# TomBeacock/volumetric-renderer

Hardware: AMD Instinct MI355X
Metric: Gsamples/sec + fps, 512³ NRRD @ 1080p; achieved HBM GB/s vs peak (higher is better)
Workload: dtype f32

## Files before the change

include/vr/vr.h:

```cpp
#ifndef VR_VR_H
#define VR_VR_H

#include <stddef.h>
#include <stdint.h>

#ifdef __cplusplus
extern "C" {
#endif

#define VR_ABI_VERSION 9

#define VR_OK 0
#define VR_EINVAL (-22)
#define VR_ENOMEM (-12)
#define VR_ENODEV (-19)
#define VR_ENODATA (-61)
#define VR_EIO (-5)

enum vr_dtype {
    VR_DTYPE_I8 = 1,
    VR_DTYPE_U8 = 2,
    VR_DTYPE_I16 = 3,
    VR_DTYPE_U16 = 4,
    VR_DTYPE_I32 = 5,
// ... 31 lines not shown
    int32_t skip_empty;
    int32_t wave_shape;
    int32_t frames_in_flight;
    int32_t exact_gradient;
    int32_t depth_zero_to_one;
} vr_params;

typedef struct vr_stats {
    uint64_t rays;
    uint64_t samples;
    uint64_t shaded_samples;
    uint64_t steps;
    uint64_t skipped_samples;
} vr_stats;

int vr_abi_version(void);
void vr_params_default(vr_params *p);

typedef struct vr_ctx vr_ctx;
vr_ctx *vr_create(int device, uint32_t width, uint32_t height);
vr_ctx *vr_create_mask(uint32_t device_mask, uint32_t width, uint32_t height);
void vr_destroy(vr_ctx *ctx);
const char *vr_last_error(const vr_ctx *ctx);

int vr_resize(vr_ctx *ctx, uint32_t width, uint32_t height);
int vr_get_size(const vr_ctx *ctx, uint32_t *width, uint32_t *height);
int vr_get_device(const vr_ctx *ctx, int *device);
int vr_get_device_mask(const vr_ctx *ctx, uint32_t *device_mask);


int vr_set_volume(vr_ctx *ctx, const void *data, int dtype, uint32_t nx, uint32_t ny,
                  uint32_t nz, float vmin, float vmax);
int vr_set_volume_device(vr_ctx *ctx, const void *data_dev, int dtype, uint32_t nx,
                         uint32_t ny, uint32_t nz, float vmin, float vmax, void *stream);
int vr_generate_volume(vr_ctx *ctx, int kind, int dtype, uint32_t nx, uint32_t ny,
                       uint32_t nz, uint32_t seed, float *vmin_out, float *vmax_out);
uint64_t vr_volume_bytes(const vr_ctx *ctx);
int vr_debug_read_volume(vr_ctx *ctx, float *out_host);
int vr_debug_read_volume_native(vr_ctx *ctx, void *out_host);
int vr_debug_volume_info(const vr_ctx *ctx, uint32_t dims[3], float minmax[2], int *storage);

int vr_set_transfer_function(vr_ctx *ctx, const uint32_t *rgba8_srgb, uint32_t n);

int vr_set_slicing(vr_ctx *ctx, const float min_slice[3], const float max_slice[3]);


int vr_render(vr_ctx *ctx, const vr_camera *cam, const vr_params *p, void *out,
              int out_format);

int vr_render_device(vr_ctx *ctx, const vr_camera *cam, const vr_params *p, void *out_dev,
                     int out_format, uint32_t row_block, uint32_t rank, uint32_t nranks,
                     void *stream);
uint32_t vr_shard_rows(uint32_t height, uint32_t row_block, uint32_t nranks);
int vr_set_row_share(vr_ctx *ctx, uint32_t first_weight, uint32_t other_weight);
int vr_get_row_share(const vr_ctx *ctx, uint32_t *first_weight, uint32_t *other_weight);
uint32_t vr_shard_rows_ctx(const vr_ctx *ctx, uint32_t height, uint32_t row_block, uint32_t nranks);
int vr_assemble_rows(vr_ctx *ctx, const void *gathered_dev, void *out_dev, int out_format,
                     uint32_t row_block, uint32_t nranks, void *stream);

typedef struct vr_external_memory vr_external_memory;
int vr_import_memory_fd(vr_ctx *ctx, int fd, uint64_t size, uint64_t offset,
                        vr_external_memory **mem, void **dev_ptr);
int vr_release_external_memory(vr_ctx *ctx, vr_external_memory *mem);

typedef struct vr_memory_info {
    uint64_t volume_bytes;
    uint64_t field_bytes;
    uint64_t oblique_copy_bytes;
    uint64_t plain_copy_bytes;
    uint64_t stencil_copy_bytes;
    uint64_t skip_bytes;
    uint64_t derived_bytes;
    uint64_t budget_bytes;
    uint64_t builds;
    uint64_t evictions;
    uint64_t downgrades;
    uint64_t last_downgrade;
} vr_memory_info;
enum vr_derived {
    VR_DERIVED_FIELD = 1,
    VR_DERIVED_OBLIQUE_COPY = 2,
    VR_DERIVED_PLAIN_COPY = 3,
    VR_DERIVED_STENCIL_COPY = 4,
    VR_DERIVED_SKIP = 5
};
#define VR_MEMORY_BUDGET_UNLIMITED (~(uint64_t)0)
#define VR_MEMORY_BUDGET_DEFAULT (~(uint64_t)0 - 1)
int vr_set_memory_budget(vr_ctx *ctx, uint64_t bytes);
int vr_memory_report(const vr_ctx *ctx, vr_memory_info *out);
int vr_prepare(vr_ctx *ctx, const vr_camera *cam, const vr_params *p);

int vr_count_work(vr_ctx *ctx, const vr_camera *cam, const vr_params *p, uint32_t row_block,
                  uint32_t rank, uint32_t nranks, vr_stats *out);

int vr_timing_enable(vr_ctx *ctx, int enable);
int vr_timing_read(vr_ctx *ctx, double *total_ms, uint64_t *launches);
int vr_timing_reset(vr_ctx *ctx);

const char *vr_kernel_name(const vr_ctx *ctx, const vr_params *p);

#ifdef __cplusplus
}
#endif

#endif
```

include/vr/vr_debug.h:

```cpp
#ifndef VR_VR_DEBUG_H
#define VR_VR_DEBUG_H

#include "vr.h"
#include "vr_dist.h"

#ifdef __cplusplus
extern "C" {
#endif

enum vr_knob {
    VR_KNOB_PIPELINE = 1,
    VR_KNOB_PAIR = 2,
    VR_KNOB_PAIR_LANES = 3,
    VR_KNOB_GRAD_FIELD = 4,
    VR_KNOB_U8_LAYOUT = 6,
    VR_KNOB_TILE_ORDER = 7,
    VR_KNOB_NARROW = 8,
    VR_KNOB_ALT_GEOMETRY = 9,
    VR_KNOB_MIP_INFLIGHT = 10
};

typedef struct vr_member_timing {
    int32_t device;
    uint64_t frames;
    double kernel_ms, render_ms, gather_ms, assemble_ms;
} vr_member_timing;
int vr_debug_timing_member(vr_ctx *ctx, int member, vr_member_timing *out);

enum vr_exchange { VR_EXCHANGE_RCCL = 0, VR_EXCHANGE_COPY = 1 };
vr_ctx *vr_debug_create_members(const int *devices, int n, uint32_t width, uint32_t height,
                                int exchange);
int vr_debug_fail_member(vr_ctx *ctx, int member, uint64_t frame);

int vr_debug_host_profile_enable(vr_ctx *ctx, int enable);
int vr_debug_host_profile_member(vr_ctx *ctx, int member, vr_dist_host_profile *out);

int vr_debug_set_knob(vr_ctx *ctx, int knob, int value);
int vr_debug_get_knob(const vr_ctx *ctx, int knob, int *value);

typedef struct vr_variant_facts {
    int32_t layout, mode;
    int32_t shade, count, skip, field, field_half, pipeline;
    int32_t tf_n, pair, mip_inflight;
} vr_variant_facts;
int vr_debug_variant_name(const vr_variant_facts *facts, char *buf, size_t n);
const char *vr_debug_last_kernel_name(const vr_ctx *ctx);

#ifdef __cplusplus
}
#endif

#endif
```

volumetric-renderer_amd/csrc/vr_api.hip:

```cpp
#include "../../include/vr/vr.h"
#include "../../include/vr/vr_debug.h"
#include "../../include/vr/vr_modes.h"
#include "../../include/vr/vr_iso.h"
#include "vr_internal.h"
#include "vr_group.h"

#include <algorithm>
#include <cmath>
#include <cstdio>
#include <cstdlib>
#include <cstring>
#include <new>
#include <string>
#include <vector>

#pragma clang fp contract(off)

using namespace vr;

#ifndef VR_HOST_BANDS
#define VR_HOST_BANDS 4
#endif
constexpr int kRenderBands = VR_HOST_BANDS;

struct vr_ctx {
    int device = 0;
    uint32_t width = 0, height = 0;
    void *bricks = nullptr;
    size_t brick_bytes = 0;
    int storage = ST_F32;
    int layout = ST_F32;
    bool dense_rows = false;
    double pixel_span = 0.0;
    double axis_align = 1.0;
    int ray_axis = 2;
    double row_align = 1.0;
    struct AltCopy {
        void *bricks = nullptr;
        size_t bytes = 0;
        bool valid = false, failed = false;
        uint64_t used = 0;
    } alt[3];
    uint32_t nx = 1, ny = 1, nz = 1;
    float vmin = 0.0f, vmax = 1.0f;
    float4 *tf = nullptr;
    uint32_t tf_n = 0;
    uint32_t *tf_nz = nullptr;
    float smin[3] = {0.0f, 0.0f, 0.0f};
    float smax[3] = {1.0f, 1.0f, 1.0f};
    int render_mode = VR_MODE_COMPOSITE;
    float isovalue = 0.0f;
    float2 *brick_range = nullptr;
    uint8_t *skip_dist = nullptr;
    size_t nbricks_alloc = 0;
    bool range_valid = false, dist_valid = false;
    float *grad = nullptr;
    size_t grad_bytes = 0;
    bool grad_valid = false;
    uint64_t grad_used = 0;
    bool grad_half = false;
    int grad_scale_log2 = 0;
    float data_lo = 0.0f, data_hi = 1.0f;
    struct TileSched {
        uint32_t tiles_x = 0, tiles_y = 0, supers_x = 0, per_xcd = 0;
        uint32_t row_block = 0, rank = 0, nranks = 0, share_w0 = 1, share_w = 1;
        int pair = 0;
        uint32_t kernel = 0;
        void *stream = nullptr;
        uint32_t *cost = nullptr, *perm = nullptr, *lists = nullptr;
        bool have_perm = false;
        uint32_t launches = 0;
    };
    std::vector<TileSched> sched;
    hipEvent_t built_ev = nullptr;
    bool built_recorded = false;
    struct Fence {
        hipStream_t stream;
        hipEvent_t ev;
        uint64_t used;
        bool external;
        uint64_t build_seen;
    };
    std::vector<Fence> fences;
    uint64_t build_gen = 0;
    uint64_t frame_no = 0;
    FrameVariant last_variant;
    uint64_t n_builds = 0, n_evictions = 0, n_downgrades = 0;
    uint32_t last_downgrade = 0;
    unsigned long long *counters = nullptr;
    void *frame_dev = nullptr;
    size_t frame_bytes = 0;
    hipStream_t band_stream[2] = {nullptr, nullptr};
    hipStream_t copy_stream = nullptr;
    hipEvent_t band_ev[kRenderBands] = {};
    bool timing = false;
    std::vector<hipEvent_t> ev_pool;
    std::vector<std::pair<hipEvent_t, hipEvent_t>> ev_pending;
    double timed_ms = 0.0;
    uint64_t timed_launches = 0;
    struct Knobs {
        int pipeline = -1, pair = -1, pair_lanes = 0, grad_field = -1, u8_layout = -1,
            tile_order = 0, narrow = 1, alt = -1, mip_inflight = 0;
    } knobs;
    std::vector<vr_ctx *> members;
    vr::Group *group = nullptr;
    uint32_t device_mask = 0;
    hipStream_t group_stream = nullptr;
    RowShare share{1, 1};
    uint64_t budget = VR_MEMORY_BUDGET_DEFAULT;
    std::string err;
};

namespace {

thread_local std::string g_err;

int fail(vr_ctx *c, int code, const std::string &msg)
{
    if (c)
        c->err = msg;
    else
        g_err = msg;
    return code;
}

// ... 312 lines not shown
}

int check_params(vr_ctx *c, const vr_params *p)
{
    if (!p) return fail(c, VR_EINVAL, "params is NULL");
    if (!(p->step > 0.0f) || !std::isfinite(p->step))
        return fail(c, VR_EINVAL, "params.step must be a positive finite float");
    if (!(p->ray_dist >= 0.0f) || !std::isfinite(p->ray_dist))
        return fail(c, VR_EINVAL, "params.ray_dist must be finite and >= 0");
    if (p->spec_power < 0 || p->spec_power > 256)
        return fail(c, VR_EINVAL, "params.spec_power must be in [0, 256]");
    if (p->frames_in_flight < 0 || p->frames_in_flight > 16)
        return fail(c, VR_EINVAL, "params.frames_in_flight must be in [0, 16]");
    if (p->exact_gradient != 0 && p->exact_gradient != 1)
        return fail(c, VR_EINVAL, "params.exact_gradient must be 0 or 1");
    if (p->depth_zero_to_one != 0 && p->depth_zero_to_one != 1)
        return fail(c, VR_EINVAL, "params.depth_zero_to_one must be 0 or 1");
    const float n = p->ray_dist / p->step;
    if (n > 1.0e8f) return fail(c, VR_EINVAL, "params.ray_dist / step too large");
    return VR_OK;
}

bool view_dense_rows(const double *inv, uint32_t W, uint32_t nx, uint32_t ny, uint32_t nz,
                     double *span, double *align, int *axis, double *row_align)
{
    *span = 0.0;
    *align = 1.0;
    *axis = 2;
    *row_align = 1.0;
    auto unproject = [&](double x, double z, double out[3]) {
        double h[4];
        for (int r = 0; r < 4; ++r) h[r] = inv[0 * 4 + r] * x + inv[2 * 4 + r] * z + inv[3 * 4 + r];
        for (int a = 0; a < 3; ++a) out[a] = h[a] / h[3];
    };
    double o[3], f[3], o2[3], f2[3], d[3], s[3];
    unproject(0.0, 0.0, o);
    unproject(0.0, 1.0, f);
    const double dx = 2.0 / (double)W;
    unproject(dx, 0.0, o2);
    unproject(dx, 1.0, f2);
    double od = 0.0, dd = 0.0;
    for (int a = 0; a < 3; ++a) {
        d[a] = f[a] - o[a];
        od += o[a] * d[a];
        dd += d[a] * d[a];
    }
    if (!(dd > 0.0)) return false;
    *align = std::fmax(std::fabs(d[0]), std::fmax(std::fabs(d[1]), std::fabs(d[2]))) / std::sqrt(dd);
    *axis = std::fabs(d[0]) >= std::fabs(d[1]) ? (std::fabs(d[0]) >= std::fabs(d[2]) ? 0 : 2)
                                               : (std::fabs(d[1]) >= std::fabs(d[2]) ? 1 : 2);
    const double t = -od / dd;
    double n2 = 0.0, v2 = 0.0;
    const double nv[3] = {(double)nx, (double)ny, (double)nz};
    for (int a = 0; a < 3; ++a) {
        s[a] = (o2[a] + t * (f2[a] - o2[a])) - (o[a] + t * d[a]);
        n2 += s[a] * s[a];
        v2 += (s[a] * nv[a]) * (s[a] * nv[a]);
    }
    if (!(n2 > 0.0)) return false;
    *span = std::sqrt(v2);
    *row_align = std::fabs(s[0]) / std::sqrt(n2);
    return *row_align >= 0.9 && *span <= 0.8;
}

constexpr double kAltAlign = 0.9, kAltSpan = 0.8, kRowsAlign = 0.97;
bool use_grad_field(const vr_ctx *c, bool half)
{
    if (c->storage != ST_F32) return false;
    if (c->knobs.grad_field >= 0) return c->knobs.grad_field == 1;
    if (c->dense_rows) return true;
    if (!half || c->axis_align < kAltAlign || c->ray_axis == 0) return false;
    return c->pixel_span <= kAltSpan || (c->ray_axis == 2 && c->row_align >= kRowsAlign);
}

bool use_pipeline(bool shading, uint32_t tiles, const vr_ctx *c)
{
    if (c->knobs.pipeline >= 0) return c->knobs.pipeline == 1;
    const size_t voxels = (size_t)c->nx * c->ny * c->nz;
    return tiles * (kThreadsPerTile / 64) < kPipelineMaxWaves ||
           c->brick_bytes >= kPipelineMinBytes || voxels >= kPipelineMinVoxels || c->dense_rows ||
           (shading && c->storage == ST_F32);
}

int want_alt(const vr_ctx *c, const vr_params *p, bool pair, bool field);
bool use_pair(const vr_ctx *c, const MarchParams &P, const vr_params *p)
{
    if (p->skip_empty || P.tf_n > kTfLds) return false;
    if (c->knobs.pair >= 0) return c->knobs.pair == 1;
    if (p->frames_in_flight >= 2) return false;
    if (!p->shading) return false;
    if (P.tiles_x * P.tiles_y * (kThreadsPerTile / 64) < kPairMaxWaves) return true;
    if (c->knobs.alt >= 0 || c->layout != ST_F32 || c->dense_rows || c->pixel_span <= kAltSpan ||
        (c->ray_axis == 2 && c->axis_align >= kAltAlign))
        return false;
    return want_alt(c, p, P.pair != 0, P.grad != nullptr) == (ST_F32 | kAltFlag);
}

int build_params(vr_ctx *c, const vr_camera *cam, const vr_params *p, void *out,
                 int out_format, uint32_t row_block, uint32_t rank, uint32_t nranks,
                 RowShare share, MarchParams &P)
{
    if (!cam) return fail(c, VR_EINVAL, "camera is NULL");
    int rc = check_params(c, p);
    if (rc) return rc;
    if (out_format != VR_OUT_RGBA8 && out_format != VR_OUT_RGBA32F)
        return fail(c, VR_EINVAL, "unknown out_format");
    if (nranks == 0 || rank >= nranks || row_block == 0)
        return fail(c, VR_EINVAL, "bad shard (row_block, rank, nranks)");
    std::memset(&P, 0, sizeof(P));
    if (!unprojection(cam, c->width, c->height, p->depth_zero_to_one != 0, P.inv))
        return fail(c, VR_EINVAL, "proj * view is singular");
    P.vol = c->bricks;
    P.vol_bytes = c->brick_bytes;
    P.tf = c->tf;
    P.out = out;
    P.counters = c->counters;
    P.fw = (double)c->width;
    P.fh = (double)c->height;
    P.nx = c->nx;
    P.ny = c->ny;
    P.nz = c->nz;
    P.nbx = bricks_for(c->nx, 0, c->layout);
    P.nby = bricks_for(c->ny, 1, c->layout);
    P.fnx = (float)c->nx;
    P.fny = (float)c->ny;
    P.fnz = (float)c->nz;
    P.vmin = c->vmin;
    P.range = c->vmax - c->vmin;
    P.div_fast = P.range >= 0x1p-40f && P.range < 0x1p100f && std::fabs(c->vmin) < 0x1p100f &&
                 std::fabs(c->vmax) < 0x1p100f;
    P.inv_range = P.div_fast ? 1.0f / P.range : 0.0f;
    P.tf_n = (int32_t)c->tf_n;
    P.tf_nf = (float)c->tf_n;
    for (int a = 0; a < 3; ++a) {
        P.smin[a] = c->smin[a];
        P.smax[a] = c->smax[a];
        P.cam[a] = cam->position[a];
    }
    P.step = p->step;
    P.nsteps = (int32_t)(p->ray_dist / p->step);
    P.ert_eps = p->ert_eps;
    for (int k = 0; k < 4; ++k) P.clear[k] = p->clear_color[k];
    P.ka = p->ambient;
    P.kd = p->diffuse;
    P.ks = p->specular;
    P.spec_power = p->spec_power;
    P.W = c->width;
    P.H = c->height;
    P.row_block = row_block;
    P.rank = rank;
    P.nranks = nranks;
    P.local_rows = share_shard_rows(c->height, row_block, nranks, share);
    P.out_bytes = (unsigned long long)P.local_rows * c->width * (out_format == VR_OUT_RGBA32F ? 16 : 4);
    P.share_w0 = share.w0;
    P.share_w = share.w;
    P.tiles_x = (c->width + 15) / 16;
    P.tiles_y = (P.local_rows + kMarchRows - 1) / kMarchRows;
    P.tile_order = p->tile_order >= 1 && p->tile_order <= 4 ? (uint32_t)p->tile_order : 4u;
    if (p->tile_order == 0 && c->knobs.tile_order >= 1)
        P.tile_order = (uint32_t)c->knobs.tile_order;
    P.wave_w_shift = p->wave_shape == 1 ? 3u : (p->wave_shape == 3 ? 2u : 4u);
    while ((64u >> P.wave_w_shift) > kMarchRows) ++P.wave_w_shift;
    P.supers_x = (P.tiles_x + kSuper - 1) / kSuper;
    P.supers_total = P.supers_x * ((P.tiles_y + kSuper - 1) / kSuper);
    P.out_format = out_format;
    P.slab_default = c->smin[0] == 0.0f && c->smin[1] == 0.0f && c->smin[2] == 0.0f &&
                     c->smax[0] == 1.0f && c->smax[1] == 1.0f && c->smax[2] == 1.0f;
    c->dense_rows = view_dense_rows(P.inv, c->width, c->nx, c->ny, c->nz, &c->pixel_span,
                                    &c->axis_align, &c->ray_axis, &c->row_align);
    P.pipelined = use_pipeline(p->shading != 0, P.tiles_x * P.tiles_y, c);
    return VR_OK;
}

vr_ctx::Fence *fence_of(vr_ctx *c, hipStream_t s)
{
    for (auto &x : c->fences)
        if (x.stream == s) return &x;
    return nullptr;
// ... 6 lines not shown
    c->built_recorded = true;
    ++c->build_gen;
    if (vr_ctx::Fence *f = fence_of(c, s)) f->build_seen = c->build_gen;
    return VR_OK;
}

constexpr size_t kSkipBytesPerBrick = sizeof(float2) + 2;
size_t derived_bytes(const vr_ctx *c)
{
    size_t b = c->grad ? c->grad_bytes : 0;
    for (const auto &a : c->alt)
        if (a.bricks) b += a.bytes + kBrickSlackBytes;
    return b + c->nbricks_alloc * kSkipBytesPerBrick;
}
constexpr uint64_t kDerivedBudgetBricks = 5;
uint64_t effective_budget(const vr_ctx *c)
{
    if (c->budget != VR_MEMORY_BUDGET_DEFAULT) return c->budget;
    return kDerivedBudgetBricks * (uint64_t)c->brick_bytes + (uint64_t)c->brick_bytes / 32 +
           64ull * kBrickSlackBytes;
}
bool budget_allows(const vr_ctx *c, size_t extra, size_t replaced)
{
    if (c->budget == VR_MEMORY_BUDGET_UNLIMITED) return true;
    const size_t now = derived_bytes(c) - replaced;
    return now + extra <= effective_budget(c);
}
constexpr size_t kMaxFences = 32;
#ifndef VR_FENCE_SYSTEM_SCOPE
#define VR_FENCE_SYSTEM_SCOPE 0
#endif
constexpr unsigned kFenceEventFlags =
    hipEventDisableTiming | (VR_FENCE_SYSTEM_SCOPE ? 0u : (unsigned)hipEventDisableSystemFence);
int fence_record(vr_ctx *c, hipStream_t s)
{
    vr_ctx::Fence *f = fence_of(c, s);
    if (f && f->external) {
        f->used = c->frame_no;
        return VR_OK;
    }
    if (!f) {
        if (c->fences.size() < kMaxFences) {
            hipEvent_t e = nullptr;
            HIP_TRY(c, hipEventCreateWithFlags(&e, kFenceEventFlags), "hipEventCreate(fence)");
            c->fences.push_back(vr_ctx::Fence{s, e, 0, false, 0});
            f = &c->fences.back();
        } else {
            vr_ctx::Fence *old = nullptr;
            for (auto &x : c->fences)
                if (!x.external && (!old || x.used < old->used)) old = &x;
            if (!old) return VR_OK;
            HIP_TRY(c, hipEventSynchronize(old->ev), "hipEventSynchronize(fence)");
            old->stream = s;
            old->build_seen = 0;
            f = old;
        }
    }
    f->used = c->frame_no;
    HIP_TRY(c, hipEventRecord(f->ev, s), "hipEventRecord(fence)");
    return VR_OK;
}
int fence_others(vr_ctx *c, hipStream_t s)
{
    for (const auto &x : c->fences)
        if (x.stream != s && hipStreamWaitEvent(s, x.ev, 0) != hipSuccess) {
            (void)hipGetLastError();
            HIP_TRY(c, hipDeviceSynchronize(), "hipDeviceSynchronize (fence fallback)");
            for (size_t i = c->fences.size(); i-- > 0;)
                if (!c->fences[i].external) {
                    hipEventDestroy(c->fences[i].ev);
                    c->fences.erase(c->fences.begin() + (long)i);
                }
            return VR_OK;
        }
    return VR_OK;
}
int release_async(vr_ctx *c, void *p, hipStream_t s)
{
    if (!p) return VR_OK;
    if (int rc = fence_others(c, s)) return rc;
    HIP_TRY(c, hipFreeAsync(p, s), "hipFreeAsync(derived structure)");
    return VR_OK;
}
int make_room(vr_ctx *c, size_t extra, size_t replaced, int keep_alt, bool keep_field, hipStream_t s,
              bool *fits)
{
    *fits = budget_allows(c, extra, replaced);
    while (!*fits) {
        int pick = -2;
        uint64_t oldest = ~0ull;
        if (c->grad && !keep_field && c->grad_used < oldest) {
            pick = -1;
            oldest = c->grad_used;
        }
        for (int i = 0; i < (int)(sizeof c->alt / sizeof c->alt[0]); ++i)
            if (i != keep_alt && c->alt[i].bricks && c->alt[i].used < oldest) {
                pick = i;
                oldest = c->alt[i].used;
            }
        if (pick == -2) return VR_OK;
        if (pick == -1) {
            if (int rc = release_async(c, c->grad, s)) return rc;
            c->grad = nullptr;
            c->grad_bytes = 0;
            c->grad_valid = false;
        } else {
            if (int rc = release_async(c, c->alt[pick].bricks, s)) return rc;
            c->alt[pick] = vr_ctx::AltCopy();
        }
        ++c->n_evictions;
        *fits = budget_allows(c, extra, replaced);
    }
    return VR_OK;
}
void free_derived(vr_ctx *c)
{
    if (c->grad) (void)hipFreeAsync(c->grad, nullptr);
    c->grad = nullptr;
    c->grad_bytes = 0;
    c->grad_valid = false;
    for (auto &a : c->alt) {
        if (a.bricks) (void)hipFreeAsync(a.bricks, nullptr);
        a = vr_ctx::AltCopy();
    }
    if (c->brick_range) hipFree(c->brick_range);
    if (c->skip_dist) hipFree(c->skip_dist);
    c->brick_range = nullptr;
    c->skip_dist = nullptr;
    c->nbricks_alloc = 0;
    c->range_valid = c->dist_valid = false;
    (void)hipStreamSynchronize(nullptr);
}

int alloc_skip(vr_ctx *c, size_t nb, bool *have)
{
    *have = false;
    if (nb > 0xFFFFFFFFull) return fail(c, VR_EINVAL, "skip_empty: too many bricks");
    if (c->nbricks_alloc != nb && !budget_allows(c, nb * kSkipBytesPerBrick, c->nbricks_alloc * kSkipBytesPerBrick))
        return VR_OK;
    if (c->nbricks_alloc != nb) {
        if (c->brick_range) hipFree(c->brick_range);
        if (c->skip_dist) hipFree(c->skip_dist);
        c->brick_range = nullptr;
        c->skip_dist = nullptr;
        c->nbricks_alloc = 0;
        c->range_valid = c->dist_valid = false;
        HIP_TRY(c, hipMalloc(&c->brick_range, (nb + 1) * sizeof(float2)), "hipMalloc(brick ranges)");
        HIP_TRY(c, hipMalloc(&c->skip_dist, 2 * nb), "hipMalloc(skip distance field)");
        c->nbricks_alloc = nb;
    }
    *have = true;
    return VR_OK;
}
int build_ranges(vr_ctx *c, size_t nb, hipStream_t s)
{
    if (c->range_valid) return VR_OK;
    HIP_TRY(c, launch_brick_range(c->layout, c->bricks, bricks_for(c->nx, 0, c->layout), bricks_for(c->ny, 1, c->layout),
                                  bricks_for(c->nz, 2, c->layout), c->brick_range, s),
            "brick range kernel");
    HIP_TRY(c, launch_range_max(c->brick_range, (uint32_t)nb, s), "brick range maximum kernel");
    c->range_valid = true;
    c->dist_valid = false;
    return VR_OK;
}
size_t brick_count(const vr_ctx *c)
{
    return (size_t)bricks_for(c->nx, 0, c->layout) * bricks_for(c->ny, 1, c->layout) * bricks_for(c->nz, 2, c->layout);
}

int ensure_skip(vr_ctx *c, MarchParams &P, hipStream_t s)
{
    const size_t nb = brick_count(c);
    bool have = false;
    if (int rc = alloc_skip(c, nb, &have)) return rc;
    if (!have) return VR_OK;
    if (!c->range_valid || !c->dist_valid) ++c->n_builds;
    if (int rc = build_ranges(c, nb, s)) return rc;
    if (!c->dist_valid) {
        HIP_TRY(c, launch_skip_dist(c->brick_range, bricks_for(c->nx, 0, c->layout), bricks_for(c->ny, 1, c->layout),
                                    bricks_for(c->nz, 2, c->layout), c->tf_nz, (int)c->tf_n, c->vmin,
                                    c->vmax - c->vmin, c->skip_dist, c->skip_dist + nb, s),
                "skip distance kernels");
// ... 55 lines not shown
        if (launch_grad_field(static_cast<const float *>(c->bricks), c->grad, c->nx, c->ny, c->nz,
                              half, k, s) != hipSuccess)
            return built;
        built = true;
        ++c->n_builds;
        c->grad_valid = true;
        c->grad_half = half;
        c->grad_scale_log2 = k;
    }
    *refused = false;
    P.grad = c->grad;
    P.grad_half = half ? 1 : 0;
    c->grad_used = c->frame_no;
    return built;
}

int wait_builds(vr_ctx *c, hipStream_t s)
{
    if (c->built_recorded) {
        vr_ctx::Fence *f = fence_of(c, s);
        if (!f || f->build_seen != c->build_gen) {
            HIP_TRY(c, hipStreamWaitEvent(s, c->built_ev, 0), "hipStreamWaitEvent(build)");
            if (f) f->build_seen = c->build_gen;
        }
    }
    return VR_OK;
}
int ensure_derived(vr_ctx *c, const vr_params *p, MarchParams &P, hipStream_t s, uint32_t *refused)
{
    if (int rc = wait_builds(c, s)) return rc;
    const bool r0 = c->range_valid, d0 = c->dist_valid;
    if (p->skip_empty) {
        int rc = ensure_skip(c, P, s);
        if (rc) return rc;
        if (!P.skip_empty) *refused = VR_DERIVED_SKIP;
    }
    bool g_refused = false;
    const bool g_built = p->shading && ensure_grad(c, P, s, p->exact_gradient == 0, &g_refused);
    if (g_refused) *refused = VR_DERIVED_FIELD;
    const bool built = (!r0 && c->range_valid) || (!d0 && c->dist_valid) || g_built;
    if (built) return record_build(c, s);
    return VR_OK;
}

int ensure_mip(vr_ctx *c, const vr_params *p, MarchParams &P, MipArgs &M, hipStream_t s,
               uint32_t *refused)
{
    if (int rc = wait_builds(c, s)) return rc;
    M.brick_range = nullptr;
    M.nbricks = 0;
    P.pipelined = 0;
    if (!p->skip_empty) return VR_OK;
    const bool r0 = c->range_valid;
    if (int rc = ensure_mip_ranges(c, P, M, s)) return rc;
    if (!P.skip_empty) *refused = VR_DERIVED_SKIP;
    if (!r0 && c->range_valid) return record_build(c, s);
    return VR_OK;
}
int mip_inflight(const vr_ctx *c, bool skip)
{
    if (c->knobs.mip_inflight) return c->knobs.mip_inflight;
    if (c->layout == ST_F32 && c->pixel_span > kAltSpan) return skip ? 4 : 1;
    if ((c->layout & kQuadFlag) && skip) return 4;
    return kMipDefaultInFlight;
}

int iso_inflight(const vr_ctx *c, bool skip)
{
    if (c->knobs.mip_inflight) return c->knobs.mip_inflight;
    if (c->layout == ST_F32 && c->pixel_span > kAltSpan) return skip ? 4 : 1;
    if (c->layout == ST_U16 || c->layout == ST_I16) return mip_inflight(c, skip);
    if (c->layout & kQuadFlag) return 4;
    return skip ? 2 : 4;
}
bool range_mode(const vr_ctx *c)
{
    return c->render_mode == VR_MODE_MIP || c->render_mode == VR_MODE_ISO;
}
IsoArgs iso_args(const vr_ctx *c, const vr_params *p, const MipArgs &M)
{
    return {M.brick_range, M.nbricks, c->isovalue, p->shading != 0};
}

int want_alt(const vr_ctx *c, const vr_params *p, bool pair, bool field)
{
    if (c->layout != ST_F32 || p->skip_empty || pair || field) return c->layout;
    int which = 0;
    if (c->knobs.alt >= 0)
        which = c->knobs.alt;
    else if (!c->dense_rows) {
        if (c->pixel_span > kAltSpan && c->row_align >= kRowsAlign)
            which = p->shading ? 4 : 3;
        else if (c->axis_align >= kAltAlign && c->ray_axis != 0 && c->pixel_span <= kAltSpan)
            which = 0;
        else
            which = 1;
    }
    switch (which) {
        case 1: return ST_F32 | kAltFlag;
        case 3: return ST_F32 | kPlainF32Flag;
        case 4: return ST_F32 | kStencilF32Flag;
        default: return c->layout;
    }
}

int alt_index(int layout)
{
    if (layout & kAltFlag) return 0;
    return (layout & kPlainF32Flag) ? 1 : 2;
}

size_t alt_bytes_for(const vr_ctx *c, int lay)
{
    return (size_t)bricks_for(c->nx, 0, lay) * bricks_for(c->ny, 1, lay) * bricks_for(c->nz, 2, lay) *
           brick_elems(lay) * element_size(lay);
}

int ensure_alt(vr_ctx *c, int lay, hipStream_t s, bool *ready)
{
    *ready = false;
    vr_ctx::AltCopy &a = c->alt[alt_index(lay)];
    const size_t bytes = alt_bytes_for(c, lay);
    if (a.valid && a.bricks && a.bytes == bytes) {
        *ready = true;
        a.used = c->frame_no;
        return VR_OK;
    }
    if (a.failed) return VR_OK;
    if (!a.bricks || a.bytes != bytes) {
        const size_t had = a.bricks ? a.bytes + kBrickSlackBytes : 0;
        bool fits = false;
        if (int rc = make_room(c, bytes + kBrickSlackBytes, had, alt_index(lay), false, s, &fits))
            return rc;
        if (!fits) return VR_OK;
        if (int rc = release_async(c, a.bricks, s)) return rc;
        a.bricks = nullptr;
        a.bytes = 0;
        size_t free_b = 0, total_b = 0;
        if (hipMemGetInfo(&free_b, &total_b) != hipSuccess ||
            free_b < bytes + kBrickSlackBytes + (2ull << 30) ||
            hipMallocAsync(&a.bricks, bytes + kBrickSlackBytes, s) != hipSuccess) {
            (void)hipGetLastError();
            a.bricks = nullptr;
            a.failed = true;
            return VR_OK;
        }
        a.bytes = bytes;
    }
    const hipError_t e = launch_rebrick_f32(static_cast<const float *>(c->bricks), a.bricks, c->nx,
                                            c->ny, c->nz, lay, s);
    if (e != hipSuccess) return hip_fail(c, e, "alt geometry copy");
    a.valid = true;
    a.used = c->frame_no;
    ++c->n_builds;
    *ready = true;
    return record_build(c, s);
}

VariantFacts launch_facts(const vr_ctx *c, const vr_params *p, const MarchParams &P, int layout,
                          bool count)
{
    const bool skip = P.skip_empty != 0;
    const int k = c->render_mode == VR_MODE_MIP   ? mip_inflight(c, skip)
                  : c->render_mode == VR_MODE_ISO ? iso_inflight(c, skip)
                                                  : 0;
    return {layout, c->render_mode, p->shading != 0, count, skip, P.grad != nullptr, P.grad_half,
            P.pipelined, P.tf_n, P.pair, k};
}
VariantFacts next_frame_facts(const vr_ctx *c, const vr_params *p)
{
    VariantFacts f{};
    f.layout = c->layout;
    f.mode = c->render_mode;
    f.shade = p && p->shading;
    f.tf_n = (int32_t)c->tf_n;
    if (range_mode(c)) {
        f.skip = p && p->skip_empty && c->range_valid && c->nbricks_alloc;
        f.mip_inflight = f.mode == VR_MODE_ISO ? iso_inflight(c, f.skip) : mip_inflight(c, f.skip);
        return f;
    }
    f.skip = p && p->skip_empty;
    f.field = f.shade && use_grad_field(c, p->exact_gradient == 0) && c->grad && c->grad_valid;
    f.field_half = f.field && p->exact_gradient == 0;
    const uint32_t tiles = ((c->width + 15) / 16) * ((c->height + kMarchRows - 1) / kMarchRows);
    f.pipeline = use_pipeline(f.shade, tiles, c);
    if (p && !f.field)
        if (const int lay = want_alt(c, p, false, false);
            lay != c->layout && c->alt[alt_index(lay)].valid)
            f.layout = lay;
    return f;
}

vr_ctx::TileSched *tile_sched(vr_ctx *c, MarchParams &P, void *stream, uint32_t kernel)
{
    if (P.tile_order != 4) return nullptr;
    auto use = [&P](vr_ctx::TileSched &t) {
        P.tile_cost = t.cost;
        if (t.have_perm) {
            P.tile_perm = t.perm;
            P.nperm = 8 * t.per_xcd;
        }
    };
    for (auto &t : c->sched)
        if (t.tiles_x == P.tiles_x && t.tiles_y == P.tiles_y && t.pair == P.pair &&
            t.kernel == kernel &&
            t.stream == stream && t.row_block == P.row_block && t.rank == P.rank &&
            t.nranks == P.nranks && t.share_w0 == P.share_w0 && t.share_w == P.share_w) {
            use(t);
            return &t;
        }
    if (c->sched.size() >= kMaxTileScheds) {
        hipFree(c->sched.front().cost);
        hipFree(c->sched.front().perm);
        hipFree(c->sched.front().lists);
        c->sched.erase(c->sched.begin());
    }
    vr_ctx::TileSched t;
    t.tiles_x = P.tiles_x;
    t.tiles_y = P.tiles_y;
    t.supers_x = P.supers_x;
    t.pair = P.pair;
    t.kernel = kernel;
    t.stream = stream;
    t.row_block = P.row_block;
    t.rank = P.rank;
    t.nranks = P.nranks;
    t.share_w0 = P.share_w0;
    t.share_w = P.share_w;
    std::vector<std::vector<uint32_t>> xl(8);
    if (VR_LIST_ORDER == 1) {
        const uint32_t sy_n = (P.tiles_y + kSuper - 1) / kSuper;
        for (uint32_t sy = 0; sy < sy_n; ++sy)
            for (uint32_t sx = 0; sx < P.supers_x; ++sx)
                for (uint32_t w = 0; w < kSuper * kSuper; ++w) {
                    const uint32_t tx = sx * kSuper + w % kSuper, ty = sy * kSuper + w / kSuper;
                    if (tx < P.tiles_x && ty < P.tiles_y)
                        xl[(sy * P.supers_x + sx) & 7u].push_back(ty * P.tiles_x + tx);
                }
    } else {
        for (uint32_t ty = 0; ty < P.tiles_y; ++ty)
            for (uint32_t tx = 0; tx < P.tiles_x; ++tx)
                xl[((ty >> kSuperShift) * P.supers_x + (tx >> kSuperShift)) & 7u].push_back(
                    ty * P.tiles_x + tx);
    }
    for (int x = 0; x < 8; ++x) t.per_xcd = xl[x].size() > t.per_xcd ? (uint32_t)xl[x].size() : t.per_xcd;
    std::vector<uint32_t> lists(8 * (size_t)t.per_xcd, 0xFFFFFFFFu);
    for (int x = 0; x < 8; ++x)
        std::copy(xl[x].begin(), xl[x].end(), lists.begin() + (size_t)x * t.per_xcd);
    const size_t nt = (size_t)P.tiles_x * P.tiles_y;
    hipStream_t hs = static_cast<hipStream_t>(stream);
    if (hipMalloc(&t.cost, nt * sizeof(uint32_t)) != hipSuccess ||
        hipMalloc(&t.perm, lists.size() * sizeof(uint32_t)) != hipSuccess ||
        hipMalloc(&t.lists, lists.size() * sizeof(uint32_t)) != hipSuccess ||
        hipMemcpyAsync(t.lists, lists.data(), lists.size() * sizeof(uint32_t),
                       hipMemcpyHostToDevice, hs) != hipSuccess) {
        (void)hipGetLastError();
        hipFree(t.cost);
        hipFree(t.perm);
        hipFree(t.lists);
        return nullptr;
    }
    c->sched.push_back(t);
    use(c->sched.back());
    return &c->sched.back();
}

bool is_group(const vr_ctx *c) { return c && c->group; }

int group_idle(vr_ctx *c)
{
    std::string m;
    if (vr::group_synchronize(c->group, &m) != VR_OK) return fail(c, VR_EIO, m);
    return VR_OK;
}

int replicate_volume(vr_ctx *c)
{
    vr_ctx *src = c->members[0];
    const size_t n = c->members.size();
    std::vector<hipStream_t> st(n, nullptr);
    int rc = VR_OK;
    for (size_t k = 1; k < n && rc == VR_OK; ++k) {
        vr_ctx *d = c->members[k];
        if ((rc = wait_idle(d)) != VR_OK) break;
        void *dst = nullptr;
        if ((rc = set_bricks(d, src->layout, src->nx, src->ny, src->nz, &dst)) != VR_OK) break;
        hipError_t e = hipStreamCreateWithFlags(&st[k], hipStreamNonBlocking);
        if (e == hipSuccess)
            e = hipMemcpyPeerAsync(dst, d->device, src->bricks, src->device, src->brick_bytes, st[k]);
        if (e != hipSuccess) rc = hip_fail(c, e, "replicate volume (peer copy)");
        if (rc == VR_OK) {
            d->storage = src->storage;
            d->layout = src->layout;
            d->nx = src->nx;
            d->ny = src->ny;
            d->nz = src->nz;
            d->vmin = src->vmin;
            d->vmax = src->vmax;
            d->data_lo = src->data_lo;
            d->data_hi = src->data_hi;
            d->range_valid = d->dist_valid = d->grad_valid = false;
        }
    }
    for (size_t k = 1; k < n; ++k)
        if (st[k]) {
            hipSetDevice(c->members[k]->device);
            const hipError_t e = hipStreamSynchronize(st[k]);
            if (e != hipSuccess && rc == VR_OK) rc = hip_fail(c, e, "replicate volume (sync)");
            hipStreamDestroy(st[k]);
        }
    hipSetDevice(c->device);
    return rc;
}

int member_rc(vr_ctx *c, vr_ctx *m, int rc)
{
    if (rc != VR_OK) c->err = m->err;
    return rc;
}

int *knob_slot(vr_ctx *c, int knob)
{
    switch (knob) {
        case VR_KNOB_PIPELINE: return &c->knobs.pipeline;
        case VR_KNOB_PAIR: return &c->knobs.pair;
        case VR_KNOB_PAIR_LANES: return &c->knobs.pair_lanes;
        case VR_KNOB_GRAD_FIELD: return &c->knobs.grad_field;
        case VR_KNOB_U8_LAYOUT: return &c->knobs.u8_layout;
        case VR_KNOB_TILE_ORDER: return &c->knobs.tile_order;
        case VR_KNOB_NARROW: return &c->knobs.narrow;
        case VR_KNOB_ALT_GEOMETRY: return &c->knobs.alt;
        case VR_KNOB_MIP_INFLIGHT: return &c->knobs.mip_inflight;
        default: return nullptr;
    }
}

bool knob_value_ok(int knob, int v)
{
    switch (knob) {
        case VR_KNOB_PAIR_LANES: return v == 0 || v == 2 || v == 4;
        case VR_KNOB_NARROW: return v == 0 || v == 1;
        case VR_KNOB_ALT_GEOMETRY: return v >= -1 && v <= 4 && v != 2;
        case VR_KNOB_TILE_ORDER: return v >= 0 && v <= 4;
        case VR_KNOB_MIP_INFLIGHT: return v == 0 || v == 1 || v == 2 || v == 4;
        default: return v >= -1 && v <= 1;
    }
}

#ifdef VR_EXPERIMENTS
void knobs_from_env(vr_ctx *c)
{
    auto flag = [](const char *name, int &dst) {
        if (const char *e = std::getenv(name)) dst = e[0] == '1' ? 1 : 0;
    };
    flag("VR_PIPELINE", c->knobs.pipeline);
    flag("VR_PAIR", c->knobs.pair);
    if (const char *e = std::getenv("VR_PAIR_LANES")) c->knobs.pair_lanes = e[0] == '4' ? 4 : 2;
    if (std::getenv("VR_NO_GRAD_FIELD")) c->knobs.grad_field = 0;
    if (std::getenv("VR_GRAD_FIELD_ALWAYS")) c->knobs.grad_field = 1;
    if (const char *e = std::getenv("VR_U8_LAYOUT")) c->knobs.u8_layout = e[0] == 'q' ? 1 : 0;
    if (const char *e = std::getenv("VR_TILE_ORDER_DEFAULT"))
        if (e[0] >= '1' && e[0] <= '4') c->knobs.tile_order = e[0] - '0';
}
#endif

hipEvent_t pooled_event(vr_ctx *c)
{
    if (!c->ev_pool.empty()) {
        hipEvent_t e = c->ev_pool.back();
        c->ev_pool.pop_back();
        return e;
    }
    hipEvent_t e = nullptr;
    if (hipEventCreateWithFlags(&e, hipEventDisableSystemFence) != hipSuccess) return nullptr;
    return e;
}

vr_ctx *create_members(const std::vector<int> &devices, uint32_t width, uint32_t height,
                       int exchange)
{
    if (width == 0 || height == 0) {
        fail(nullptr, VR_EINVAL, "framebuffer size must be non-zero");
        return nullptr;
    }
    vr_ctx *c = new (std::nothrow) vr_ctx();
    if (!c) {
        fail(nullptr, VR_ENOMEM, "out of host memory");
        return nullptr;
    }
    c->device = devices[0];
    for (int d : devices)
        if (d < 32) c->device_mask |= 1u << d;
    c->width = width;
    c->height = height;
#ifdef VR_EXPERIMENTS
    knobs_from_env(c);
#endif
    for (int d : devices) {
        vr_ctx *m = vr_create(d, width, height);
        if (!m) {
            const std::string e = g_err;
            vr_destroy(c);
            fail(nullptr, VR_ENODEV, "device " + std::to_string(d) + ": " + e);
            return nullptr;
        }
        m->knobs = c->knobs;
        c->members.push_back(m);
    }
    std::string err;
    c->group = vr::group_create(c->members, exchange, &err);
    if (!c->group) {
        vr_destroy(c);
        fail(nullptr, VR_ENODEV, "multi-device context: " + err);
        return nullptr;
    }
    hipSetDevice(c->device);
    return c;
}

}

bool vr::is_multi_device(const vr_ctx *c) { return is_group(c); }

int vr::register_stream_fence(vr_ctx *c, hipStream_t stream, hipEvent_t ev)
{
// ... 596 lines not shown
    uint64_t *copies[3] = {&out->oblique_copy_bytes, &out->plain_copy_bytes, &out->stencil_copy_bytes};
    for (int i = 0; i < 3; ++i)
        *copies[i] = c->alt[i].bricks ? c->alt[i].bytes + kBrickSlackBytes : 0;
    out->skip_bytes = c->nbricks_alloc * kSkipBytesPerBrick;
    out->derived_bytes = derived_bytes(c);
    out->budget_bytes = c->budget == VR_MEMORY_BUDGET_UNLIMITED ? c->budget : effective_budget(c);
    out->builds = c->n_builds;
    out->evictions = c->n_evictions;
    out->downgrades = c->n_downgrades;
    out->last_downgrade = c->last_downgrade;
    return VR_OK;
}

int vr_prepare(vr_ctx *c, const vr_camera *cam, const vr_params *p)
{
    if (!c) return fail(nullptr, VR_EINVAL, "ctx is NULL");
    if (is_group(c)) {
        if (int rc = group_idle(c)) return rc;
        for (vr_ctx *m : c->members)
            if (int rc = vr_prepare(m, cam, p)) return member_rc(c, m, rc);
        hipSetDevice(c->device);
        return VR_OK;
    }
    HIP_TRY(c, hipSetDevice(c->device), "hipSetDevice");
    if (int rc = render_device_impl(c, cam, p, c->counters, VR_OUT_RGBA8, 16, 0, 1, c->share,
                                    nullptr, false))
        return rc;
    HIP_TRY(c, hipStreamSynchronize(nullptr), "hipStreamSynchronize (prepare)");
    return VR_OK;
}

int vr_render_device(vr_ctx *c, const vr_camera *cam, const vr_params *p, void *out_dev,
                     int out_format, uint32_t row_block, uint32_t rank, uint32_t nranks,
                     void *stream)
{
    if (!c) return fail(nullptr, VR_EINVAL, "ctx is NULL");
    return render_device_impl(c, cam, p, out_dev, out_format, row_block, rank, nranks, c->share,
                              stream);
}

}
namespace {
int render_device_impl(vr_ctx *c, const vr_camera *cam, const vr_params *p, void *out_dev,
                       int out_format, uint32_t row_block, uint32_t rank, uint32_t nranks,
                       RowShare share, void *stream, bool launch)
{
    if (!out_dev) return fail(c, VR_EINVAL, "output buffer is NULL");
    if (is_group(c)) {
        if (rank != 0 || nranks != 1)
            return fail(c, VR_EINVAL, "a multi-device context renders whole frames (rank 0 of 1)");
        if (!cam) return fail(c, VR_EINVAL, "camera is NULL");
        if (int rc = check_params(c, p)) return rc;
        if (out_format != VR_OUT_RGBA8 && out_format != VR_OUT_RGBA32F)
            return fail(c, VR_EINVAL, "unknown out_format");
        std::string m;
        if (int rc = vr::group_render(c->group, cam, p, out_dev, out_format,
                                      static_cast<hipStream_t>(stream), &m))
            return fail(c, rc, m);
        return VR_OK;
    }
    MarchParams P;
    int rc = build_params(c, cam, p, out_dev, out_format, row_block, rank, nranks, share, P);
    if (rc) return rc;
    HIP_TRY(c, hipSetDevice(c->device), "hipSetDevice");
    hipStream_t s = static_cast<hipStream_t>(stream);
    ++c->frame_no;
    uint32_t refused = 0;
    MipArgs M{nullptr, 0};
    int layout = c->layout;
    const bool mip = range_mode(c);
    if (mip) {
        rc = ensure_mip(c, p, P, M, s, &refused);
        if (rc) return rc;
    } else {
        rc = ensure_derived(c, p, P, s, &refused);
        if (rc) return rc;
        if (use_pair(c, P, p)) {
            P.pair = P.tiles_x * P.tiles_y * (kThreadsPerTile / 64) < kPairQuadMaxWaves ? 4 : 2;
            if (c->knobs.pair_lanes == 2 || c->knobs.pair_lanes == 4) P.pair = c->knobs.pair_lanes;
            const uint32_t th = 16 / P.pair;
            P.tiles_y = (P.local_rows + th - 1) / th;
            P.supers_total = P.supers_x * ((P.tiles_y + kSuper - 1) / kSuper);
        }
        if (const int lay = want_alt(c, p, P.pair != 0, P.grad != nullptr); lay != c->layout) {
            bool ready = false;
            rc = ensure_alt(c, lay, s, &ready);
            if (rc) return rc;
            if (ready) {
                layout = lay;
                P.vol = c->alt[alt_index(lay)].bricks;
                P.vol_bytes = c->alt[alt_index(lay)].bytes;
                P.nbx = bricks_for(c->nx, 0, layout);
                P.nby = bricks_for(c->ny, 1, layout);
            } else {
                refused = (uint32_t)(VR_DERIVED_OBLIQUE_COPY + alt_index(lay));
            }
        }
    }
    if (!launch) return VR_OK;
    if (refused) {
        ++c->n_downgrades;
        c->last_downgrade = refused;
    }
    FrameVariant v;
    resolve_variant(launch_facts(c, p, P, layout, false), &v);
    vr_ctx::TileSched *ts = tile_sched(c, P, stream, variant_tile_key(v, layout));
    hipEvent_t e0 = nullptr, e1 = nullptr;
    const bool timing = c->timing;
    if (timing) {
        e0 = pooled_event(c);
        e1 = pooled_event(c);
        if (!e0 || !e1) return fail(c, VR_EIO, "hipEventCreate failed");
        HIP_TRY(c, hipEventRecord(e0, s), "hipEventRecord");
    }
    HIP_TRY(c, launch_frame(v, P, M, iso_args(c, p, M), s),
            v.family == VF_ISO ? "iso kernel launch" : mip ? "mip kernel launch" : "march kernel launch");
    c->last_variant = v;
    if (timing) {
        HIP_TRY(c, hipEventRecord(e1, s), "hipEventRecord");
        c->ev_pending.emplace_back(e0, e1);
    }
    if (ts && ts->launches++ % kReorderEvery == 0) {
        HIP_TRY(c, launch_order_tiles(ts->cost, ts->lists, ts->perm, ts->per_xcd, s),
                "tile order kernel");
        ts->have_perm = true;
    }
    return fence_record(c, s);
}
}
extern "C" {

int vr_render(vr_ctx *c, const vr_camera *cam, const vr_params *p, void *out, int out_format)
{
    if (!c) return fail(nullptr, VR_EINVAL, "ctx is NULL");
    if (!out) return fail(c, VR_EINVAL, "output buffer is NULL");
    if (!p) return fail(c, VR_EINVAL, "params is NULL");
    HIP_TRY(c, hipSetDevice(c->device), "hipSetDevice");
    const size_t bpp = out_format == VR_OUT_RGBA32F ? 16 : 4;
    const uint32_t W = c->width, H = c->height;
    if (is_group(c)) {
        const size_t fb = (size_t)W * H * bpp;
        if (c->frame_bytes < fb) {
            if (c->frame_dev) hipFree(c->frame_dev);
            c->frame_dev = nullptr;
            c->frame_bytes = 0;
            HIP_TRY(c, hipMalloc(&c->frame_dev, fb), "hipMalloc(frame)");
            c->frame_bytes = fb;
        }
        if (!c->group_stream)
            HIP_TRY(c, hipStreamCreateWithFlags(&c->group_stream, hipStreamNonBlocking),
                    "hipStreamCreate");
        int rc = vr_render_device(c, cam, p, c->frame_dev, out_format, vr::kGroupRowBlock, 0, 1,
                                  c->group_stream);
        if (rc) return rc;
        HIP_TRY(c, hipMemcpyAsync(out, c->frame_dev, fb, hipMemcpyDeviceToHost, c->group_stream),
                "hipMemcpyAsync(frame)");
        HIP_TRY(c, hipStreamSynchronize(c->group_stream), "hipStreamSynchronize(frame)");
        return VR_OK;
    }
    const int nb = H >= kHostBandMinRows ? kRenderBands : 1;
    const uint32_t R = nb == 1 ? 16 : ((H + nb - 1) / nb + 15) / 16 * 16;
    const size_t bytes = (size_t)W * (nb == 1 ? H : (size_t)R * nb) * bpp;
    if (c->frame_bytes < bytes) {
        if (c->frame_dev) hipFree(c->frame_dev);
        c->frame_dev = nullptr;
        c->frame_bytes = 0;
        HIP_TRY(c, hipMalloc(&c->frame_dev, bytes), "hipMalloc(frame)");
        c->frame_bytes = bytes;
    }
    if (nb == 1) {
        int rc = render_device_impl(c, cam, p, c->frame_dev, out_format, 16, 0, 1, RowShare{1, 1},
                                    nullptr);
        if (rc) return rc;
        HIP_TRY(c, hipMemcpy(out, c->frame_dev, (size_t)W * H * bpp, hipMemcpyDeviceToHost),
                "hipMemcpy(frame)");
        return VR_OK;
    }
    if (!c->copy_stream) {
// ... 215 lines not shown
    if (!c) return fail(nullptr, VR_EINVAL, "ctx is NULL");
    if (is_group(c)) {
        if (int rc = group_idle(c)) return rc;
        double ms = 0.0;
        uint64_t n = 0;
        for (vr_ctx *m : c->members) {
            double a = 0.0;
            uint64_t b = 0;
            if (int rc = vr_timing_read(m, &a, &b)) return member_rc(c, m, rc);
            ms += a;
            n += b;
        }
        hipSetDevice(c->device);
        if (total_ms) *total_ms = ms;
        if (launches) *launches = n;
        return VR_OK;
    }
    HIP_TRY(c, hipSetDevice(c->device), "hipSetDevice");
    for (auto &pr : c->ev_pending) {
        if (hipEventSynchronize(pr.second) != hipSuccess) {
            (void)hipGetLastError();
            HIP_TRY(c, hipDeviceSynchronize(), "hipDeviceSynchronize (timing)");
        }
        float ms = 0.0f;
        HIP_TRY(c, hipEventElapsedTime(&ms, pr.first, pr.second), "hipEventElapsedTime");
        c->timed_ms += ms;
        c->timed_launches++;
        c->ev_pool.push_back(pr.first);
        c->ev_pool.push_back(pr.second);
    }
    c->ev_pending.clear();
    if (total_ms) *total_ms = c->timed_ms;
    if (launches) *launches = c->timed_launches;
    return VR_OK;
}

int vr_timing_reset(vr_ctx *c)
{
    if (is_group(c)) {
        if (int rc = group_idle(c)) return rc;
        std::string m;
        if (int rc = vr::group_timing_reset(c->group, &m)) return fail(c, rc, m);
        for (vr_ctx *m : c->members)
            if (int rc = vr_timing_reset(m)) return member_rc(c, m, rc);
        return VR_OK;
    }
    double ms;
    uint64_t n;
    int rc = vr_timing_read(c, &ms, &n);
    if (rc) return rc;
    c->timed_ms = 0.0;
    c->timed_launches = 0;
    return VR_OK;
}

const char *vr_kernel_name(const vr_ctx *c, const vr_params *p)
{
    if (!c) return "";
    if (is_group(c)) return vr_kernel_name(c->members[0], p);
    thread_local std::string name;
    FrameVariant v;
    resolve_variant(next_frame_facts(c, p), &v);
    name = variant_kernel_name(v);
    return name.c_str();
}

int vr_debug_variant_name(const vr_variant_facts *facts, char *buf, size_t n)
{
    FrameVariant v;
    if (!facts || !buf || n == 0 || !resolve_variant(*facts, &v)) return VR_EINVAL;
    std::snprintf(buf, n, "%s", variant_kernel_name(v).c_str());
    return VR_OK;
}

const char *vr_debug_last_kernel_name(const vr_ctx *c)
{
    if (!c) return "";
    if (is_group(c)) return vr_debug_last_kernel_name(c->members[0]);
    thread_local std::string name;
    name = variant_kernel_name(c->last_variant);
    return name.c_str();
}

int vr_debug_set_knob(vr_ctx *c, int knob, int value)
{
    if (!c) return fail(nullptr, VR_EINVAL, "ctx is NULL");
    int *k = knob_slot(c, knob);
    if (!k) return fail(c, VR_EINVAL, "unknown knob");
    if (!knob_value_ok(knob, value)) return fail(c, VR_EINVAL, "knob value out of range");
    if (is_group(c))
        if (int rc = group_idle(c)) return rc;
    *k = value;
    for (vr_ctx *m : c->members) vr_debug_set_knob(m, knob, value);
    return VR_OK;
}

int vr_debug_get_knob(const vr_ctx *c, int knob, int *value)
{
    if (!c || !value) return fail(nullptr, VR_EINVAL, "NULL argument");
    int *k = knob_slot(const_cast<vr_ctx *>(c), knob);
    if (!k) return fail(nullptr, VR_EINVAL, "unknown knob");
    *value = *k;
    return VR_OK;
}

#ifdef VR_WG_TIMES
int vr_debug_wg_times(unsigned long long *out, unsigned int max, unsigned int *count, int reset)
{
    if (reset) return debug_wg_times_reset() == hipSuccess ? VR_OK : VR_EIO;
    return debug_wg_times_read(out, max, count) == hipSuccess ? VR_OK : VR_EIO;
}
#endif

}
```

volumetric-renderer_amd/csrc/vr_internal.h:

```cpp
#pragma once

#include <hip/hip_runtime.h>
#include <stddef.h>
#include <stdint.h>

#include <cmath>
#include <type_traits>

#include "vr_variant.h"

namespace vr {

#ifndef VR_BRICK_CELLS
#define VR_BRICK_CELLS 8, 8, 8
#endif
#ifndef VR_BRICK_ALIGN
#define VR_BRICK_ALIGN 1
#endif
template <int X, int Y, int Z, int LO = 0>
struct BrickGeom {
    static constexpr int BX = X, BY = Y, BZ = Z;
    static constexpr int Lo = LO;
    static constexpr int EX = X + 1 + 2 * LO, EY = Y + 1 + 2 * LO, EZ = Z + 1 + 2 * LO;
    static constexpr int Row = EX, Slice = EX * EY;
    static constexpr int Elems = (EX * EY * EZ + VR_BRICK_ALIGN - 1) / VR_BRICK_ALIGN * VR_BRICK_ALIGN;
    __host__ __device__ static constexpr int cells(int a) { return a == 0 ? X : (a == 1 ? Y : Z); }
};
using GeomWide = BrickGeom<VR_BRICK_CELLS>;
#ifndef VR_U8_PLAIN
#define VR_U8_PLAIN 1
#endif
#ifndef VR_U8_BRICK_CELLS
#define VR_U8_BRICK_CELLS 7, 8, 8
#endif
using GeomByte = std::conditional_t<VR_U8_PLAIN != 0, BrickGeom<VR_U8_BRICK_CELLS>, GeomWide>;
constexpr size_t kBrickSlackBytes = 64;
#ifndef VR_F32_PLAIN
#define VR_F32_PLAIN 0
#endif
constexpr size_t kF32VoxelsPerElement = VR_F32_PLAIN ? 1 : 2;
constexpr int kPad = 2;

#ifndef VR_BRICK_GROUP_SHIFT
#define VR_BRICK_GROUP_SHIFT 0
#endif
constexpr int kGroupShift = VR_BRICK_GROUP_SHIFT;
constexpr uint32_t kGroupMask = (1u << kGroupShift) - 1;

__host__ __device__ __forceinline__ uint32_t morton_spread(uint32_t v)
{
    uint32_t r = 0;
#pragma unroll
    for (int t = 0; t < kGroupShift; ++t) r |= ((v >> t) & 1u) << (3 * t);
    return r;
}

__host__ __device__ __forceinline__ uint32_t brick_slot(uint32_t bx, uint32_t by, uint32_t bz,
                                                        uint32_t nbx, uint32_t nby)
{
    if constexpr (kGroupShift == 0) {
        return (bz * nby + by) * nbx + bx;
    } else {
        constexpr uint32_t G = kGroupShift;
        const uint32_t grp = ((bz >> G) * (nby >> G) + (by >> G)) * (nbx >> G) + (bx >> G);
        return (grp << (3 * G)) | morton_spread(bx & kGroupMask) |
               (morton_spread(by & kGroupMask) << 1) | (morton_spread(bz & kGroupMask) << 2);
    }
}

__host__ __device__ __forceinline__ void brick_coords(uint32_t slot, uint32_t nbx, uint32_t nby,
                                                      uint32_t &bx, uint32_t &by, uint32_t &bz)
{
    if constexpr (kGroupShift == 0) {
        bx = slot % nbx;
        by = (slot / nbx) % nby;
        bz = slot / (nbx * nby);
    } else {
        constexpr uint32_t G = kGroupShift;
        const uint32_t grp = slot >> (3 * G), m = slot & ((1u << (3 * G)) - 1);
        const uint32_t gx = nbx >> G, gy = nby >> G;
        uint32_t lx = 0, ly = 0, lz = 0;
#pragma unroll
        for (int t = 0; t < (int)G; ++t) {
            lx |= ((m >> (3 * t)) & 1u) << t;
            ly |= ((m >> (3 * t + 1)) & 1u) << t;
            lz |= ((m >> (3 * t + 2)) & 1u) << t;
        }
        bx = ((grp % gx) << G) | lx;
        by = (((grp / gx) % gy) << G) | ly;
        bz = ((grp / (gx * gy)) << G) | lz;
    }
}

constexpr size_t kQuadMaxVoxels = 1ull << 25;
template <typename T>
struct Quad8 {
    T v;
};
#ifndef VR_ALT_BRICK_CELLS
#define VR_ALT_BRICK_CELLS 7, 15, 8
#endif
using GeomAlt = BrickGeom<VR_ALT_BRICK_CELLS>;
struct F32Alt {
    float v;
};
#ifndef VR_PLAIN_BRICK_CELLS
#define VR_PLAIN_BRICK_CELLS 15, 15, 15
#endif
using GeomPlainRows = BrickGeom<VR_PLAIN_BRICK_CELLS>;
struct F32P {
    float v;
};
#ifndef VR_STENCIL_BRICK_CELLS
#define VR_STENCIL_BRICK_CELLS 29, 29, 29
#endif
using GeomStencil = BrickGeom<VR_STENCIL_BRICK_CELLS, 1>;
struct F32S {
    float v;
};
struct F32H {
    float v;
};

inline size_t storage_size(int st)
{
    switch (st & 0xF) {
        case ST_U8:
        case ST_I8: return 1;
        case ST_U16:
        case ST_I16: return 2;
        default: return 4;
    }
}
inline bool byte_storage(int st)
{
    return VR_U8_PLAIN && !(st & kQuadFlag) && (st == ST_U8 || st == ST_I8);
}
inline size_t voxels_per_element(int st)
{
    if (st & (kPlainF32Flag | kStencilF32Flag)) return 1;
    return (st & 0xF) == ST_F32 ? kF32VoxelsPerElement : (byte_storage(st) ? 1 : 4);
}
inline size_t element_size(int st) { return storage_size(st) * voxels_per_element(st); }
inline int brick_cells(int st, int a)
{
    if (st & kAltFlag) return GeomAlt::cells(a);
    if (st & kPlainF32Flag) return GeomPlainRows::cells(a);
    if (st & kStencilF32Flag) return GeomStencil::cells(a);
    return byte_storage(st) ? GeomByte::cells(a) : GeomWide::cells(a);
}
inline size_t brick_elems(int st)
{
    if (st & kAltFlag) return GeomAlt::Elems;
    if (st & kPlainF32Flag) return GeomPlainRows::Elems;
    if (st & kStencilF32Flag) return GeomStencil::Elems;
    return byte_storage(st) ? GeomByte::Elems : GeomWide::Elems;
}

inline uint32_t bricks_for(uint32_t n, int a, int st)
{
    return ((n + 3) / (uint32_t)brick_cells(st, a) + 1 + kGroupMask) & ~kGroupMask;
}

struct RowShare {
    uint32_t w0, w;
};
__host__ __device__ inline uint32_t share_period(uint32_t n, RowShare s) { return s.w0 + (n - 1) * s.w; }
__host__ __device__ inline uint32_t share_offset(uint32_t r, RowShare s)
{
    return r == 0 ? 0u : s.w0 + (r - 1) * s.w;
}
__host__ __device__ inline uint32_t share_global_block(uint32_t lb, uint32_t r, uint32_t n, RowShare s)
{
    const uint32_t w = r == 0 ? s.w0 : s.w;
    return (lb / w) * share_period(n, s) + share_offset(r, s) + lb % w;
}
__host__ __device__ inline void share_owner(uint32_t gb, uint32_t n, RowShare s, uint32_t &r,
                                            uint32_t &lb)
{
    const uint32_t P = share_period(n, s), q = gb / P, o = gb - q * P;
    if (o < s.w0) {
        r = 0;
        lb = q * s.w0 + o;
    } else {
        const uint32_t t = o - s.w0;
        r = 1 + t / s.w;
        lb = q * s.w + t % s.w;
    }
}
inline uint32_t share_blocks(uint32_t nb, uint32_t r, uint32_t n, RowShare s)
{
    const uint32_t P = share_period(n, s), q = nb / P, o = nb - q * P;
    const uint32_t w = r == 0 ? s.w0 : s.w, off = share_offset(r, s);
    const uint32_t tail = o > off ? (o - off < w ? o - off : w) : 0u;
    return q * w + tail;
}
inline uint32_t share_shard_rows(uint32_t height, uint32_t row_block, uint32_t n, RowShare s)
{
    if (row_block == 0 || n == 0 || s.w0 == 0 || s.w == 0) return 0;
    const uint32_t nb = (height + row_block - 1) / row_block;
    uint32_t m = share_blocks(nb, 0, n, s);
    if (n > 1) {
        const uint32_t b1 = share_blocks(nb, 1, n, s);
        m = b1 > m ? b1 : m;
    }
// ... 135 lines not shown
```

volumetric-renderer_amd/csrc/vr_kernels.hip:

```cpp
#include "vr_exact_math.h"
#include "vr_internal.h"

#include <array>
#include <cstdlib>
#include <tuple>
#include <type_traits>
#include <utility>

#pragma clang fp contract(off)

namespace vr {
namespace {

constexpr int kTile = 16;
constexpr int kThreads = 256;
constexpr int kTfLut = 2 * (kTfLds + 2);

__device__ __forceinline__ float lerpf(float a, float b, float w) { return fmaf(w, b - a, a); }

#ifdef VR_BOUNDS_CHECK
__device__ unsigned int g_oob_reports;
__device__ __noinline__ void oob_report(int what, unsigned long long a, unsigned long long b)
{
    if (atomicAdd(&g_oob_reports, 1u) < 32u)
        printf("VR_OOB what=%d index=%llu limit=%llu block=%u thread=%u\n", what, a, b,
               (unsigned)blockIdx.x, (unsigned)threadIdx.x);
}
#define VR_OOB(what, a, b) ((unsigned long long)(a) >= (unsigned long long)(b) ? (oob_report((what), (a), (b)), true) : false)
#else
#define VR_OOB(what, a, b) false
#endif

typedef float f2v __attribute__((ext_vector_type(2)));
__device__ __forceinline__ f2v lerp2(f2v a, f2v b, float w)
{
    const f2v ww = {w, w};
    return __builtin_elementwise_fma(ww, b - a, a);
}

typedef float f2a __attribute__((ext_vector_type(2))) __attribute__((aligned(4)));
typedef float f4a __attribute__((ext_vector_type(4))) __attribute__((aligned(4)));
typedef uint32_t u2a __attribute__((ext_vector_type(2))) __attribute__((aligned(4)));
typedef uint32_t u4a __attribute__((ext_vector_type(4))) __attribute__((aligned(4)));

template <typename VT>
struct is_quad8 : std::false_type {};
template <typename T>
struct is_quad8<Quad8<T>> : std::true_type {};
template <typename VT>
struct VoxOf {
    using type = VT;
};
template <typename T>
struct VoxOf<Quad8<T>> {
    using type = T;
};
template <>
struct VoxOf<F32Alt> {
    using type = float;
};
template <>
struct VoxOf<F32H> {
    using type = float;
};
template <>
struct VoxOf<F32P> {
    using type = float;
};
template <>
struct VoxOf<F32S> {
    using type = float;
};
template <typename VT>
using Vox = typename VoxOf<VT>::type;
template <typename VT>
constexpr bool kIsQuad8 = is_quad8<VT>::value;
template <typename VT>
constexpr bool kHalfField = std::is_same<VT, F32H>::value;
template <typename VT>
constexpr bool kZPair = std::is_same<Vox<VT>, float>::value;
template <typename VT>
constexpr bool kPlainF32 = std::is_same<VT, F32P>::value || std::is_same<VT, F32S>::value ||
                          (kZPair<VT> && VR_F32_PLAIN);
template <typename VT>
constexpr bool kStencil = std::is_same<VT, F32S>::value;
#ifndef VR_STENCIL_WIDE
#define VR_STENCIL_WIDE 1
#endif
template <typename VT>
constexpr bool kStencilWide = kStencil<VT> && VR_STENCIL_WIDE;
template <typename VT>
constexpr bool kPlainByte = sizeof(VT) == 1 && VR_U8_PLAIN && !kIsQuad8<VT>;
template <typename VT>
constexpr int kElemBytes = kZPair<VT> ? (kPlainF32<VT> ? 4 : 8)
                                      : (kPlainByte<VT> ? 1 : 4 * (int)sizeof(VT));
template <typename VT>
using GeomOf = std::conditional_t<kPlainByte<VT>, GeomByte,
                                  std::conditional_t<std::is_same<VT, F32Alt>::value, GeomAlt,
                                  std::conditional_t<std::is_same<VT, F32P>::value, GeomPlainRows,
                                  std::conditional_t<kStencil<VT>, GeomStencil, GeomWide>>>>;
template <typename VT>
constexpr int kQuadWords = sizeof(VT) == 1 ? 1 : 2;

template <typename VT>
__device__ __forceinline__ size_t cell_offset(int pi, int pj, int pk, uint32_t nbx, uint32_t nby)
{
    using G = GeomOf<VT>;
    const uint32_t ux = (uint32_t)pi, uy = (uint32_t)pj, uz = (uint32_t)pk;
    const uint32_t bx = ux / G::BX, by = uy / G::BY, bz = uz / G::BZ;
    const uint32_t l = ((uz - bz * G::BZ + G::Lo) * G::EY + (uy - by * G::BY + G::Lo)) * G::EX +
                       (ux - bx * G::BX + G::Lo);
    return (size_t)brick_slot(bx, by, bz, nbx, nby) * (size_t)G::Elems + l;
}

__device__ __forceinline__ float tri8(float v000, float v100, float v010, float v110, float v001,
                                      float v101, float v011, float v111, float ax, float ay,
                                      float az)
{
    const float c00 = lerpf(v000, v100, ax);
    const float c10 = lerpf(v010, v110, ax);
    const float c01 = lerpf(v001, v101, ax);
    const float c11 = lerpf(v011, v111, ax);
    const float c0 = lerpf(c00, c10, ay);
    const float c1 = lerpf(c01, c11, ay);
    return lerpf(c0, c1, az);
}
__device__ __forceinline__ f2v tri8x2(f2v v000, f2v v100, f2v v010, f2v v110, f2v v001,
                                      f2v v101, f2v v011, f2v v111, float ax, float ay, float az)
{
    const f2v c00 = lerp2(v000, v100, ax);
    const f2v c10 = lerp2(v010, v110, ax);
    const f2v c01 = lerp2(v001, v101, ax);
    const f2v c11 = lerp2(v011, v111, ax);
    const f2v c0 = lerp2(c00, c10, ay);
    const f2v c1 = lerp2(c01, c11, ay);
    return lerp2(c0, c1, az);
}

template <typename VT>
__device__ __forceinline__ float byte_value(uint32_t w, int b)
{
    const uint32_t u = (w >> (8 * b)) & 0xFFu;
    if constexpr (std::is_signed<Vox<VT>>::value) return (float)(int)(int8_t)u;
    return (float)u;
}

template <typename VT>
__device__ __forceinline__ float qc(const uint32_t *w, int c)
{
    if constexpr (sizeof(VT) == 1) {
        const uint32_t b = (w[0] >> (8 * c)) & 0xFFu;
        if constexpr (std::is_signed<Vox<VT>>::value) return (float)(int)(int8_t)b;
        return (float)b;
    } else {
        const uint32_t h = (w[c >> 1] >> (16 * (c & 1))) & 0xFFFFu;
        if constexpr (std::is_signed<Vox<VT>>::value) return (float)(int)(int16_t)h;
        return (float)h;
    }
}

template <typename VT>
__device__ __forceinline__ void quad_load2(const char *__restrict__ base, size_t e, uint32_t *w)
{
    const char *p = base + e * kElemBytes<VT>;
    if constexpr (sizeof(VT) == 1) {
        const u2a r = *reinterpret_cast<const u2a *>(p);
        w[0] = r.x;
        w[1] = r.y;
    } else {
        const u4a r = *reinterpret_cast<const u4a *>(p);
        w[0] = r.x;
        w[1] = r.y;
        w[2] = r.z;
        w[3] = r.w;
    }
}
template <typename VT>
__device__ __forceinline__ void quad_load1(const char *__restrict__ base, size_t e, uint32_t *w)
{
    const char *p = base + e * kElemBytes<VT>;
    if constexpr (sizeof(VT) == 1) {
        w[0] = *reinterpret_cast<const uint32_t *>(p);
    } else {
        const u2a r = *reinterpret_cast<const u2a *>(p);
        w[0] = r.x;
        w[1] = r.y;
    }
}
__device__ __forceinline__ f4a zpair_load2(const char *__restrict__ base, size_t e)
{
    return *reinterpret_cast<const f4a *>(base + e * 8);
}
__device__ __forceinline__ f2a zpair_load1(const char *__restrict__ base, size_t e)
{
    return *reinterpret_cast<const f2a *>(base + e * 8);
}

template <typename VT, typename = void>
struct CellRaw {
    float v[8];
};
template <typename VT>
struct CellRaw<VT, std::enable_if_t<kZPair<VT> && !kPlainF32<VT>>> {
    f4a r0, r1;
};
template <typename VT>
struct CellRaw<VT, std::enable_if_t<kStencilWide<VT>>> {
    f4a q[4];
};
template <typename VT>
struct CellRaw<VT, std::enable_if_t<kPlainByte<VT> && GeomByte::EX == 8>> {
    u4a q0, q1;
    uint32_t sh;
};


template <typename VT, typename = void>
struct CellTaps {};
template <typename VT>
struct CellTaps<VT, std::enable_if_t<kStencilWide<VT>>> {
    float xm[4], xp[4];
};
template <typename VT>
struct Cell8 : CellTaps<VT> {
    float v[8];
    static __device__ __forceinline__ void issue(CellRaw<VT> &w, const char *__restrict__ base,
                                                 size_t e)
    {
        if constexpr (kZPair<VT> && !kPlainF32<VT>) {
            w.r0 = zpair_load2(base, e);
            w.r1 = zpair_load2(base, e + GeomOf<VT>::Row);
        } else if constexpr (kStencilWide<VT>) {
            using G = GeomOf<VT>;
#pragma unroll
            for (int r = 0; r < 4; ++r)
                w.q[r] = *reinterpret_cast<const f4a *>(
                    base + (e - 1 + (size_t)((r & 1) * G::Row + (r >> 1) * G::Slice)) * 4);
        } else if constexpr (kPlainByte<VT> && GeomByte::EX == 8) {
            const size_t a = e & ~(size_t)3;
            w.sh = (uint32_t)e & 3u;
            w.q0 = *reinterpret_cast<const u4a *>(base + a);
            w.q1 = *reinterpret_cast<const u4a *>(base + a + GeomByte::Slice);
        } else {
            Cell8 c;
            c.load(base, e);
#pragma unroll
            for (int i = 0; i < 8; ++i) w.v[i] = c.v[i];
        }
    }
    __device__ __forceinline__ void decode(const CellRaw<VT> &w)
    {
        if constexpr (kZPair<VT> && !kPlainF32<VT>) {
            v[0] = w.r0.x;
            v[4] = w.r0.y;
            v[1] = w.r0.z;
            v[5] = w.r0.w;
            v[2] = w.r1.x;
            v[6] = w.r1.y;
            v[3] = w.r1.z;
            v[7] = w.r1.w;
        } else if constexpr (kStencilWide<VT>) {
#pragma unroll
            for (int r = 0; r < 4; ++r) {
                this->xm[r] = w.q[r].x;
                v[2 * r] = w.q[r].y;
                v[2 * r + 1] = w.q[r].z;
                this->xp[r] = w.q[r].w;
            }
        } else if constexpr (kPlainByte<VT> && GeomByte::EX == 8) {
            const uint32_t q[4] = {__builtin_amdgcn_alignbyte(w.q0.y, w.q0.x, w.sh),
                                   __builtin_amdgcn_alignbyte(w.q0.w, w.q0.z, w.sh),
                                   __builtin_amdgcn_alignbyte(w.q1.y, w.q1.x, w.sh),
                                   __builtin_amdgcn_alignbyte(w.q1.w, w.q1.z, w.sh)};
#pragma unroll
            for (int r = 0; r < 4; ++r) {
                v[2 * r] = byte_value<VT>(q[r], 0);
                v[2 * r + 1] = byte_value<VT>(q[r], 1);
            }
        } else {
#pragma unroll
            for (int i = 0; i < 8; ++i) v[i] = w.v[i];
        }
    }
    __device__ __forceinline__ void load(const char *__restrict__ base, size_t e)
    {
        if constexpr (kStencilWide<VT>) {
            CellRaw<VT> w;
            issue(w, base, e);
            decode(w);
        } else if constexpr (kPlainF32<VT>) {
            using G = GeomOf<VT>;
#pragma unroll
            for (int r = 0; r < 4; ++r) {
                const f2a q = *reinterpret_cast<const f2a *>(
                    base + (e + (size_t)((r & 1) * G::Row + (r >> 1) * G::Slice)) * 4);
                v[2 * r] = q.x;
                v[2 * r + 1] = q.y;
            }
        } else if constexpr (kZPair<VT>) {
            const f4a r0 = zpair_load2(base, e);
            const f4a r1 = zpair_load2(base, e + GeomOf<VT>::Row);
            v[0] = r0.x;
            v[4] = r0.y;
            v[1] = r0.z;
            v[5] = r0.w;
            v[2] = r1.x;
            v[6] = r1.y;
            v[3] = r1.z;
            v[7] = r1.w;
        } else if constexpr (kPlainByte<VT> && GeomByte::EX == 4) {
            const size_t a = e & ~(size_t)3;
            const uint32_t sh = 8u * ((uint32_t)e & 3u);
            const u2a q0 = *reinterpret_cast<const u2a *>(base + a);
            const u2a q1 = *reinterpret_cast<const u2a *>(base + a + GeomByte::Slice);
            const uint32_t w[4] = {q0.x >> sh, q0.y >> sh, q1.x >> sh, q1.y >> sh};
#pragma unroll
            for (int r = 0; r < 4; ++r) {
                v[2 * r] = byte_value<VT>(w[r], 0);
                v[2 * r + 1] = byte_value<VT>(w[r], 1);
            }
        } else if constexpr (kPlainByte<VT>) {
            static_assert(GeomByte::EX == 8, "plain 8-bit rows are 4 or 8 bytes");
            const size_t a = e & ~(size_t)3;
            const uint32_t sh = (uint32_t)e & 3u;
            const u4a q0 = *reinterpret_cast<const u4a *>(base + a);
            const u4a q1 = *reinterpret_cast<const u4a *>(base + a + GeomByte::Slice);
            const uint32_t w[4] = {__builtin_amdgcn_alignbyte(q0.y, q0.x, sh),
                                   __builtin_amdgcn_alignbyte(q0.w, q0.z, sh),
                                   __builtin_amdgcn_alignbyte(q1.y, q1.x, sh),
                                   __builtin_amdgcn_alignbyte(q1.w, q1.z, sh)};
#pragma unroll
            for (int r = 0; r < 4; ++r) {
                v[2 * r] = byte_value<VT>(w[r], 0);
                v[2 * r + 1] = byte_value<VT>(w[r], 1);
            }
        } else {
            constexpr int QW = kQuadWords<VT>;
            uint32_t w[2 * QW];
            quad_load2<VT>(base, e, w);
            v[0] = qc<VT>(w, 0);
            v[4] = qc<VT>(w, 1);
            v[2] = qc<VT>(w, 2);
            v[6] = qc<VT>(w, 3);
            v[1] = qc<VT>(w + QW, 0);
            v[5] = qc<VT>(w + QW, 1);
            v[3] = qc<VT>(w + QW, 2);
            v[7] = qc<VT>(w + QW, 3);
        }
    }
    __device__ __forceinline__ float tri(float ax, float ay, float az) const
    {
        return tri8(v[0], v[1], v[2], v[3], v[4], v[5], v[6], v[7], ax, ay, az);
    }
};

template <bool PACKED>
__device__ __forceinline__ void grad_filter(const float *dx, const float *dy, const float *dz,
                                            float ax, float ay, float az, float &gx, float &gy,
                                            float &gz)
{
    if constexpr (PACKED) {
        const f2v g = tri8x2(f2v{dx[0], dy[0]}, f2v{dx[1], dy[1]}, f2v{dx[2], dy[2]},
                             f2v{dx[3], dy[3]}, f2v{dx[4], dy[4]}, f2v{dx[5], dy[5]},
                             f2v{dx[6], dy[6]}, f2v{dx[7], dy[7]}, ax, ay, az);
        gx = g.x;
        gy = g.y;
    } else {
        gx = tri8(dx[0], dx[1], dx[2], dx[3], dx[4], dx[5], dx[6], dx[7], ax, ay, az);
        gy = tri8(dy[0], dy[1], dy[2], dy[3], dy[4], dy[5], dy[6], dy[7], ax, ay, az);
// ... 524 lines not shown
}

template <typename VT, bool GF, bool PACKED>
__device__ __forceinline__ void shade_sample(const MarchParams &P, const char *__restrict__ vol,
                                             size_t ce, const Cell8<VT> &c, int pi, int pj,
                                             int pk, long by_stride, long bz_stride, float ax,
                                             float ay, float az, float d0, float d1, float d2,
                                             float4 &s)
{
    float gx, gy_, gz;
    if constexpr (GF) {
        grad_field<PACKED, kHalfField<VT>>(reinterpret_cast<const char *>(P.grad), ce, ax, ay, az,
                                           gx, gy_, gz);
    } else {
        gradient<VT, PACKED>(vol, ce, c, pi, pj, pk, P.nbx, P.nby, by_stride, bz_stride, ax, ay,
                             az, gx, gy_, gz);
    }
    phong(P, gx, gy_, gz, d0, d1, d2, s);
}

template <typename VT, bool SHADE, bool COUNT, bool SKIP, bool GF, bool PIPE>
__device__ __forceinline__ void march_strip(const MarchParams &P, LdsF4 *s_tf,
                                            bool tf_in_lds, uint32_t tile_x, uint32_t tile_y,
                                            uint32_t wave, uint32_t lane)
{
    using G = GeomOf<VT>;
    const long by_stride = (long)P.nbx * G::Elems;
    const long bz_stride = (long)P.nbx * P.nby * G::Elems;

    const uint32_t ws = P.wave_w_shift, ww = 1u << ws, wh = 64u >> ws;
    const uint32_t wpr = kTile >> ws;
    const uint32_t lx_ = lane & (ww - 1), ly_ = lane >> ws;
    const uint32_t px = tile_x * kTile + (wave % wpr) * ww + lx_;
    const uint32_t ly = tile_y * kMarchRows + (wave / wpr) * wh + ly_;
    bool active = px < P.W && ly < P.local_rows;
    const uint32_t blk = ly / P.row_block;
    const uint32_t gy = share_global_block(blk, P.rank, P.nranks, RowShare{P.share_w0, P.share_w}) *
                            P.row_block + (ly - blk * P.row_block);
    active = active && gy < P.H;

    float tex[3] = {0.f, 0.f, 0.f}, dir[3] = {0.f, 0.f, 0.f};
    const bool covered = active && pixel_ray(P, px, gy, tex, dir);

    float T = 1.0f, cr = 0.0f, cg = 0.0f, cb = 0.0f;
    unsigned long long n_samples = 0, n_shaded = 0, n_steps = 0, n_skipped = 0;
    uint32_t cur_brick = 0xFFFFFFFFu, cur_dist = 0;
    const char *__restrict__ vol = static_cast<const char *>(P.vol);
    const int nsteps = covered ? P.nsteps : 0;
    float p0 = tex[0], p1 = tex[1], p2 = tex[2];
    const float d0 = dir[0], d1 = dir[1], d2 = dir[2];
    const int kin = (covered && P.slab_default) ? interior_steps(tex, dir, P.step, nsteps) : 0;
    float inv_du[3] = {0.f, 0.f, 0.f}, leap_margin[3] = {0.f, 0.f, 0.f};
    if (!COUNT && SKIP) {
        const float dd[3] = {d0, d1, d2}, fn[3] = {P.fnx, P.fny, P.fnz};
#pragma unroll
        for (int a = 0; a < 3; ++a) {
            inv_du[a] = 1.0f / (fabsf(dd[a]) * P.step * fn[a]);
            leap_margin[a] = 0.5f + (float)kMaxLeap * 1.2e-7f * fn[a];
        }
    }
    if constexpr (PIPE) {
        struct Stage {
            CellRaw<VT> w;
            size_t ce;
            float ax, ay, az;
            int pi, pj, pk;
            bool ok, slab;
        };
        auto prep = [&](Stage &S, int k, bool live = true) {
            const bool interior = (unsigned)(k - 1) < (unsigned)kin;
            S.ok = live && k < nsteps &&
                   (interior || !(p0 > 1.0f || p1 > 1.0f || p2 > 1.0f || p0 < 0.0f ||
                                  p1 < 0.0f || p2 < 0.0f));
            S.slab = S.ok && (interior || (p0 < P.smax[0] && p1 < P.smax[1] && p2 < P.smax[2] &&
                                           p0 > P.smin[0] && p1 > P.smin[1] && p2 > P.smin[2]));
            int i, j, kk;
            texel_coord(p0, P.fnx, i, S.ax);
            texel_coord(p1, P.fny, j, S.ay);
            texel_coord(p2, P.fnz, kk, S.az);
            if (!S.slab) i = j = kk = 0;
            S.pi = i + kPad;
            S.pj = j + kPad;
            S.pk = kk + kPad;
            S.ce = cell_offset<VT>(S.pi, S.pj, S.pk, P.nbx, P.nby);
            if (VR_OOB(3, S.ce * kElemBytes<VT>, P.vol_bytes)) S.ce = 0;
            Cell8<VT>::issue(S.w, vol, S.ce);
        };
        auto composite = [&](const float4 &sm) -> bool {
            cr = cr + (sm.x * sm.w) * T;
            cg = cg + (sm.y * sm.w) * T;
            cb = cb + (sm.z * sm.w) * T;
            T = T * (1.0f - sm.w);
            return T == 0.0f || T < P.ert_eps;
        };
        constexpr bool kDefer = VR_DEFER_SHADE && SHADE && GF;
        struct Pend {
            FieldRowsT<kHalfField<VT>> g;
            float4 sm;
            float ax, ay, az;
            bool on;
        } X;
        X.on = false;
        auto finish = [&]() -> bool {
            if (!kDefer || !X.on) return false;
            X.on = false;
            float gx, gy_, gz;
            field_rows_filter(X.g, X.ax, X.ay, X.az, gx, gy_, gz);
            phong(P, gx, gy_, gz, d0, d1, d2, X.sm);
            return composite(X.sm);
        };
        auto consume_cell = [&](const Stage &S, const Cell8<VT> &c) -> bool {
            if (kDefer && finish()) return true;
            const float d = c.tri(S.ax, S.ay, S.az);
            const float tt = div_by_range(d - P.vmin, P);
            float4 sm = tf_lookup(s_tf, P.tf_n, P.tf_nf, tt);
            if (!S.slab) sm.w = 0.0f;
            if constexpr (kDefer) {
                if (sm.w > 0.0f) {
                    field_rows_load(reinterpret_cast<const char *>(P.grad), S.ce, X.g);
                    X.sm = sm;
                    X.ax = S.ax;
                    X.ay = S.ay;
                    X.az = S.az;
                    X.on = true;
                }
                return false;
            }
            if (SHADE && sm.w > 0.0f)
                shade_sample<VT, GF, true>(P, vol, S.ce, c, S.pi, S.pj, S.pk, by_stride,
                                           bz_stride, S.ax, S.ay, S.az, d0, d1, d2, sm);
            return composite(sm);
        };
        auto consume = [&](const Stage &S) -> bool {
            Cell8<VT> c;
            c.decode(S.w);
            return consume_cell(S, c);
        };
        auto advance = [&]() {
            p0 = p0 + d0 * P.step;
            p1 = p1 + d1 * P.step;
            p2 = p2 + d2 * P.step;
        };
        Stage A, B;
        int k = 0;
        {
            prep(A, k);
            while (A.ok) {
                advance();
                prep(B, ++k);
                if (consume(A) || !B.ok) break;
                advance();
                prep(A, ++k);
                if (consume(B)) break;
            }
        }
        finish();
    } else
    for (int it = 0; it < nsteps; ++it) {
        const bool interior = (unsigned)(it - 1) < (unsigned)kin;
        if (!interior &&
            (p0 > 1.0f || p1 > 1.0f || p2 > 1.0f || p0 < 0.0f || p1 < 0.0f || p2 < 0.0f))
            break;
        if (COUNT) ++n_steps;
        if (interior || (p0 < P.smax[0] && p1 < P.smax[1] && p2 < P.smax[2] && p0 > P.smin[0] &&
                         p1 > P.smin[1] && p2 > P.smin[2])) {
            int i, j, k;
            float ax, ay, az;
            texel_coord(p0, P.fnx, i, ax);
            texel_coord(p1, P.fny, j, ay);
// ... 42 lines not shown
                Cell8<VT> c;
                c.load(vol, ce);
                const float d = c.tri(ax, ay, az);
                const float tt = div_by_range(d - P.vmin, P);
                float4 s = tf_in_lds ? tf_lookup(s_tf, P.tf_n, P.tf_nf, tt)
                                     : tf_lookup(P.tf, P.tf_n, P.tf_nf, tt);
                if (COUNT) ++n_samples;
                if (SHADE && s.w > 0.0f) {
                    shade_sample<VT, GF, kPackedGradient<SKIP>>(P, vol, ce, c, pi, pj, pk, by_stride,
                                                                bz_stride, ax, ay, az, d0, d1, d2, s);
                    if (COUNT) ++n_shaded;
                }
                cr = cr + (s.x * s.w) * T;
                cg = cg + (s.y * s.w) * T;
                cb = cb + (s.z * s.w) * T;
                T = T * (1.0f - s.w);
                if (T == 0.0f) break;
                if (T < P.ert_eps) break;
            }
        }
        p0 = p0 + d0 * P.step;
        p1 = p1 + d1 * P.step;
        p2 = p2 + d2 * P.step;
    }

    if (COUNT) {
        const unsigned long long rays = wave_sum(covered ? 1ull : 0ull);
        const unsigned long long sm = wave_sum(n_samples);
        const unsigned long long sh = wave_sum(n_shaded);
        const unsigned long long st = wave_sum(n_steps);
        const unsigned long long sk = wave_sum(n_skipped);
        if (lane == 0) {
            atomicAdd(&P.counters[0], rays);
            atomicAdd(&P.counters[1], sm);
            atomicAdd(&P.counters[2], sh);
            atomicAdd(&P.counters[3], st);
            atomicAdd(&P.counters[4], sk);
        }
    }
    if (!active) return;

    const float A = 1.0f - T;
    const float omA = 1.0f - A;
    const float o0 = cr * A + P.clear[0] * omA;
    const float o1 = cg * A + P.clear[1] * omA;
    const float o2 = cb * A + P.clear[2] * omA;
    const float o3 = A * A + P.clear[3] * omA;
    const size_t idx = (size_t)ly * P.W + px;
    if (VR_OOB(4, idx * (P.out_format == 0 ? 4 : 16), P.out_bytes)) return;
    if (P.out_format == 0) {
        static_cast<uint32_t *>(P.out)[idx] =
            unorm8(o0) | (unorm8(o1) << 8) | (unorm8(o2) << 16) | (unorm8(o3) << 24);
    } else {
        static_cast<float4 *>(P.out)[idx] = make_float4(o0, o1, o2, o3);
    }
}

template <typename VT, bool SHADE, bool COUNT, bool SKIP, bool GF, bool PIPE>
__global__ __launch_bounds__(kThreadsPerTile, (kMarchMinWaves<COUNT, SKIP, GF, PIPE>)) void march_kernel(const MarchParams P)
{
    __shared__ float4 s_tf[kTfLut];
    const int tid = threadIdx.x;

    uint32_t tile_x, tile_y;
    if (!block_tile(P, tile_x, tile_y)) return;
    const long long wg_start = wall_clock64();

    const bool tf_in_lds = P.tf_n <= kTfLds;
    if (tf_in_lds)
        for (int i = tid; i < 2 * (P.tf_n + 2); i += (int)kThreadsPerTile) s_tf[i] = P.tf[i];
    __syncthreads();
    march_strip<VT, SHADE, COUNT, SKIP, GF, PIPE>(P, (LdsF4 *)s_tf, tf_in_lds, tile_x, tile_y,
                                                  (uint32_t)tid >> 6, (uint32_t)tid & 63u);
    if (P.tile_cost) {
        __syncthreads();
        if (tid == 0)
            P.tile_cost[tile_y * P.tiles_x + tile_x] =
                (uint32_t)min(wall_clock64() - wg_start, 0x7FFFFFFFLL);
    }
#ifdef VR_WG_TIMES
    __syncthreads();
    if (tid == 0) wg_times_record((unsigned long long)wg_start, tile_y * P.tiles_x + tile_x);
#endif
}

template <typename VT>
constexpr bool kMipQuadRaw = !kZPair<VT> && !kPlainByte<VT>;
template <typename VT, typename = void>
struct MipRaw {
    CellRaw<VT> w;
    __device__ __forceinline__ void issue(const char *__restrict__ base, size_t e)
    {
        Cell8<VT>::issue(w, base, e);
    }
    __device__ __forceinline__ void decode(Cell8<VT> &c) const { c.decode(w); }
};
template <typename VT>
struct MipRaw<VT, std::enable_if_t<kMipQuadRaw<VT>>> {
    uint32_t w[2 * kQuadWords<VT>];
    __device__ __forceinline__ void issue(const char *__restrict__ base, size_t e)
    {
        quad_load2<VT>(base, e, w);
    }
    __device__ __forceinline__ void decode(Cell8<VT> &c) const
    {
        constexpr int QW = kQuadWords<VT>;
        c.v[0] = qc<VT>(w, 0);
        c.v[4] = qc<VT>(w, 1);
        c.v[2] = qc<VT>(w, 2);
        c.v[6] = qc<VT>(w, 3);
        c.v[1] = qc<VT>(w + QW, 0);
        c.v[5] = qc<VT>(w + QW, 1);
        c.v[3] = qc<VT>(w + QW, 2);
        c.v[7] = qc<VT>(w + QW, 3);
    }
};

template <typename VT, bool COUNT, bool SKIP, int K>
__device__ __forceinline__ void mip_strip(const MarchParams &P, const MipArgs &M, uint32_t tile_x,
                                          uint32_t tile_y, uint32_t wave, uint32_t lane)
{
    using G = GeomOf<VT>;
    const uint32_t ws = P.wave_w_shift, ww = 1u << ws, wh = 64u >> ws;
    const uint32_t wpr = kTile >> ws;
    const uint32_t lx_ = lane & (ww - 1), ly_ = lane >> ws;
    const uint32_t px = tile_x * kTile + (wave % wpr) * ww + lx_;
    const uint32_t ly = tile_y * kMarchRows + (wave / wpr) * wh + ly_;
    bool active = px < P.W && ly < P.local_rows;
    const uint32_t blk = ly / P.row_block;
    const uint32_t gy = share_global_block(blk, P.rank, P.nranks, RowShare{P.share_w0, P.share_w}) *
                            P.row_block + (ly - blk * P.row_block);
    active = active && gy < P.H;

    float tex[3] = {0.f, 0.f, 0.f}, dir[3] = {0.f, 0.f, 0.f};
    const bool covered = active && pixel_ray(P, px, gy, tex, dir);

    float m = -INFINITY;
    bool any = false;
    unsigned long long n_samples = 0, n_steps = 0, n_skipped = 0;
    uint32_t cur_brick = 0xFFFFFFFFu;
    float cur_hi = INFINITY;
    const char *__restrict__ vol = static_cast<const char *>(P.vol);
    const int nsteps = covered ? P.nsteps : 0;
    float p0 = tex[0], p1 = tex[1], p2 = tex[2];
    const float d0 = dir[0], d1 = dir[1], d2 = dir[2];
    const int kin = (covered && P.slab_default) ? interior_steps(tex, dir, P.step, nsteps) : 0;
    float end_at = INFINITY;
    if constexpr (SKIP && !COUNT && !kZPair<VT>) end_at = M.brick_range[M.nbricks].y;

    struct Stage {
        MipRaw<VT> r;
        float ax, ay, az;
        bool fetch, issued;
    };
    bool live = nsteps > 0;
    for (int it = 0; live; it += K) {
        Stage S[K];
        const float m_in = m;
#pragma unroll
        for (int s = 0; s < K; ++s) {
            const int k = it + s;
            const bool interior = (unsigned)(k - 1) < (unsigned)kin;
            live = live && k < nsteps &&
                   (interior || !(p0 > 1.0f || p1 > 1.0f || p2 > 1.0f || p0 < 0.0f || p1 < 0.0f ||
                                  p2 < 0.0f));
            if (COUNT && live) ++n_steps;
// ... 642 lines not shown
            const bool ok = f >= (float)kIntRangeLo && f <= (float)kIntRangeHi && f == rintf(f) &&
                            !(f == 0.0f && signbit(f));
            bad |= ok ? 0 : 1;
            iv = ok ? (int)f : 0;
        } else {
            const bool ok = (long long)v >= kIntRangeLo && (long long)v <= kIntRangeHi &&
                            !(std::is_unsigned<SrcT>::value && (unsigned long long)v > (unsigned long long)kIntRangeHi);
            bad |= ok ? 0 : 1;
            iv = ok ? (int)v : 0;
        }
        lo = iv < lo ? iv : lo;
        hi = iv > hi ? iv : hi;
    }
#pragma unroll
    for (int off = 32; off > 0; off >>= 1) {
        const int l2 = __shfl_xor(lo, off, 64), h2 = __shfl_xor(hi, off, 64), b2 = __shfl_xor(bad, off, 64);
        lo = l2 < lo ? l2 : lo;
        hi = h2 > hi ? h2 : hi;
        bad |= b2;
    }
    __shared__ int s_lo[4], s_hi[4], s_bad[4];
    const uint32_t w = threadIdx.x >> 6;
    if ((threadIdx.x & 63) == 0) {
        s_lo[w] = lo;
        s_hi[w] = hi;
        s_bad[w] = bad;
    }
    __syncthreads();
    if (threadIdx.x == 0) {
        for (uint32_t i = 1; i < (blockDim.x >> 6); ++i) {
            lo = s_lo[i] < lo ? s_lo[i] : lo;
            hi = s_hi[i] > hi ? s_hi[i] : hi;
            bad |= s_bad[i];
        }
        atomicMin(&out[0], lo);
        atomicMax(&out[1], hi);
        if (bad) atomicOr(&out[2], 1);
    }
}


__device__ __forceinline__ float padded_voxel(const float *__restrict__ bricks, int px, int py,
                                              int pz, uint32_t nx, uint32_t ny, uint32_t nz,
                                              uint32_t nbx, uint32_t nby)
{
    if (px < kPad || py < kPad || pz < kPad || px >= (int)nx + kPad || py >= (int)ny + kPad ||
        pz >= (int)nz + kPad)
        return 0.0f;
    return bricks[kF32VoxelsPerElement * cell_offset<float>(px, py, pz, nbx, nby)];
}

template <typename DstT>
__global__ __launch_bounds__(256) void rebrick_f32_kernel(const float *__restrict__ src,
                                                          float *__restrict__ dst, uint32_t nx,
                                                          uint32_t ny, uint32_t nz, uint32_t snbx,
                                                          uint32_t snby, uint32_t snbz, uint32_t nbx,
                                                          uint32_t nby, size_t nbricks)
{
    using G = GeomOf<DstT>;
    for (size_t bidx = blockIdx.x; bidx < nbricks; bidx += gridDim.x) {
        uint32_t bx, by, bz;
        brick_coords((uint32_t)bidx, nbx, nby, bx, by, bz);
        for (uint32_t l = threadIdx.x; l < (uint32_t)G::Elems; l += blockDim.x) {
            const size_t g = bidx * G::Elems + l;
            const uint32_t lx = l % G::EX, lyz = l / G::EX, lyy = lyz % G::EY, lz = lyz / G::EY;
            const int x = (int)(bx * G::BX + lx) - G::Lo, y = (int)(by * G::BY + lyy) - G::Lo,
                      z = (int)(bz * G::BZ + lz) - G::Lo;
            if constexpr (kPlainF32<DstT>) {
                dst[g] = padded_voxel(src, x, y, z, nx, ny, nz, snbx, snby);
            } else if (kF32VoxelsPerElement == 2 && x >= 0 && y >= 0 && z >= 0 &&
                       x < (int)(snbx * GeomWide::BX) && y < (int)(snby * GeomWide::BY) &&
                       z < (int)(snbz * GeomWide::BZ)) {
                reinterpret_cast<float2 *>(dst)[g] =
                    reinterpret_cast<const float2 *>(src)[cell_offset<float>(x, y, z, snbx, snby)];
            } else {
                reinterpret_cast<float2 *>(dst)[g] =
                    make_float2(padded_voxel(src, x, y, z, nx, ny, nz, snbx, snby),
                                padded_voxel(src, x, y, z + 1, nx, ny, nz, snbx, snby));
            }
        }
    }
}

__device__ __forceinline__ _Float16 field_half(float d, float scale)
{
    float x = d * scale;
    x = x > 65504.0f ? 65504.0f : (x < -65504.0f ? -65504.0f : x);
    return (_Float16)x;
}

template <bool H>
__global__ __launch_bounds__(256) void grad_field_kernel(const float *__restrict__ bricks,
                                                         float *__restrict__ grad, uint32_t nx,
                                                         uint32_t ny, uint32_t nz, uint32_t nbx,
                                                         uint32_t nby, size_t nbricks, float scale)
{
    using G = GeomWide;
    constexpr int LX = G::EX + 2, LY = G::EY + 2 + (H ? 1 : 0), LZ = G::EZ + 3;
    __shared__ float box[LX * LY * LZ];
    __shared__ uint2 ostage[3 * G::Elems];
    uint2 *__restrict__ out = reinterpret_cast<uint2 *>(grad);
    const uint32_t nbz = (uint32_t)(nbricks / ((size_t)nbx * nby));
    for (size_t bidx = blockIdx.x; bidx < nbricks; bidx += gridDim.x) {
        uint32_t bx, by, bz;
        brick_coords((uint32_t)bidx, nbx, nby, bx, by, bz);
        const int x0 = (int)(bx * G::BX) - 1, y0 = (int)(by * G::BY) - 1, z0 = (int)(bz * G::BZ) - 1;
        __syncthreads();
        static_assert(LZ % 2 == 0, "the box is loaded in z-pairs");
        for (int i = (int)threadIdx.x; i < LX * LY * (LZ / 2); i += (int)blockDim.x) {
            const int ix = i % LX, iyz = i / LX, iy = iyz % LY, iz = 2 * (iyz / LY);
            const int px = x0 + ix, py = y0 + iy, pz = z0 + iz;
            float2 v;
            if (kF32VoxelsPerElement == 2 && px >= 0 && py >= 0 && pz >= 0 &&
                px < (int)(nbx * G::BX) && py < (int)(nby * G::BY) && pz < (int)(nbz * G::BZ))
                v = reinterpret_cast<const float2 *>(bricks)[cell_offset<float>(px, py, pz, nbx, nby)];
            else
                v = make_float2(padded_voxel(bricks, px, py, pz, nx, ny, nz, nbx, nby),
                                padded_voxel(bricks, px, py, pz + 1, nx, ny, nz, nbx, nby));
            box[(iz * LY + iy) * LX + ix] = v.x;
            box[((iz + 1) * LY + iy) * LX + ix] = v.y;
        }
        __syncthreads();
        for (uint32_t l = threadIdx.x; l < (uint32_t)G::Elems; l += blockDim.x) {
            const uint32_t lx = l % G::EX, lyz = l / G::EX, lyy = lyz % G::EY, lz = lyz / G::EY;
            uint2 *o = ostage + 3 * l;
            if (lz >= (uint32_t)G::EZ) {
                o[0] = o[1] = o[2] = make_uint2(0u, 0u);
                continue;
            }
            const int c = ((int)lz + 1) * (LX * LY) + ((int)lyy + 1) * LX + ((int)lx + 1);
            if constexpr (H) {
                _Float16 hv[12];
#pragma unroll
                for (int q = 0; q < 4; ++q) {
                    const int cq = c + (q >> 1) * LX + (q & 1) * (LX * LY);
                    auto V = [&](int dx, int dy, int dz) { return box[cq + dx + dy * LX + dz * (LX * LY)]; };
                    hv[0 + q] = field_half(V(1, 0, 0) - V(-1, 0, 0), scale);
                    hv[4 + q] = field_half(V(0, 1, 0) - V(0, -1, 0), scale);
                    hv[8 + q] = field_half(V(0, 0, 1) - V(0, 0, -1), scale);
                }
#pragma unroll
                for (int i = 0; i < 3; ++i) {
                    const h2v lo = {hv[4 * i], hv[4 * i + 1]}, hi = {hv[4 * i + 2], hv[4 * i + 3]};
                    o[i] = make_uint2(__builtin_bit_cast(uint32_t, lo), __builtin_bit_cast(uint32_t, hi));
                }
            } else {
                float d[6];
#pragma unroll
                for (int h = 0; h < 2; ++h) {
                    const int ch = c + h * (LX * LY);
                    auto V = [&](int dx, int dy, int dz) { return box[ch + dx + dy * LX + dz * (LX * LY)]; };
                    d[0 + h] = V(1, 0, 0) - V(-1, 0, 0);
                    d[2 + h] = V(0, 1, 0) - V(0, -1, 0);
                    d[4 + h] = V(0, 0, 1) - V(0, 0, -1);
                }
#pragma unroll
                for (int i = 0; i < 3; ++i)
                    o[i] = make_uint2(__float_as_uint(d[2 * i]), __float_as_uint(d[2 * i + 1]));
            }
        }
        __syncthreads();
        uint2 *__restrict__ ob = out + bidx * (3 * (size_t)G::Elems);
        for (uint32_t j = threadIdx.x; j < 3u * (uint32_t)G::Elems; j += blockDim.x) ob[j] = ostage[j];
    }
}

// ... 57 lines not shown
                                                       int tf_n, float tf_nf, float vmin,
                                                       float vrange, uint8_t *__restrict__ dist)
{
    constexpr float kRangeMargin = 4.0e-6f;
    const uint32_t b = blockIdx.x * blockDim.x + threadIdx.x;
    if (b >= nbricks) return;
    bool empty = false;
    if (vrange > 0.0f) {
        const float2 r = range[b];
        if (r.x == r.x && r.y == r.y) {
            const float m = (fabsf(r.x) + fabsf(r.y)) * kRangeMargin;
            const float t0 = ((r.x - m) - vmin) / vrange;
            const float t1 = ((r.y + m) - vmin) / vrange;
            float u0 = t0 * tf_nf - 0.5f, u1 = t1 * tf_nf - 0.5f;
            u0 = fminf(fmaxf(u0, -1.0f), tf_nf);
            u1 = fminf(fmaxf(u1, -1.0f), tf_nf);
            int i0 = (int)floorf(u0), i1 = (int)floorf(u1) + 1;
            i0 = i0 < 0 ? 0 : (i0 > tf_n - 1 ? tf_n - 1 : i0);
            i1 = i1 < 0 ? 0 : (i1 > tf_n - 1 ? tf_n - 1 : i1);
            empty = tf_nz[i1 + 1] == tf_nz[i0];
        }
    }
    dist[b] = empty ? (uint8_t)kSkipCap : (uint8_t)0;
}

__global__ __launch_bounds__(256) void dist_pass_kernel(const uint8_t *__restrict__ in,
                                                        uint8_t *__restrict__ out, uint32_t nbx,
                                                        uint32_t nby, uint32_t nbz, int axis)
{
    const uint32_t nb = nbx * nby * nbz;
    const uint32_t b = blockIdx.x * blockDim.x + threadIdx.x;
    if (b >= nb) return;
    const uint32_t bx = b % nbx, by = (b / nbx) % nby, bz = b / (nbx * nby);
    const int pos = axis == 0 ? (int)bx : (axis == 1 ? (int)by : (int)bz);
    const int len = axis == 0 ? (int)nbx : (axis == 1 ? (int)nby : (int)nbz);
    const long stride = axis == 0 ? 1 : (axis == 1 ? (long)nbx : (long)nbx * nby);
    int best = in[b];
    for (int o = 1; o < kSkipCap && o < best; ++o) {
        if (pos - o >= 0) {
            const int v = in[b - o * stride];
            best = min(best, max(o, v));
        }
        if (pos + o < len) {
            const int v = in[b + o * stride];
            best = min(best, max(o, v));
        }
    }
    out[b] = (uint8_t)best;
}


template <typename PixT>
__global__ __launch_bounds__(256) void assemble_kernel(const PixT *__restrict__ gathered,
                                                       PixT *__restrict__ out, uint32_t W,
                                                       uint32_t H, uint32_t rb, uint32_t nranks,
                                                       uint32_t shard_rows, RowShare share)
{
    const size_t total = (size_t)W * H;
    for (size_t g = (size_t)blockIdx.x * blockDim.x + threadIdx.x; g < total;
         g += (size_t)gridDim.x * blockDim.x) {
        const uint32_t y = (uint32_t)(g / W), x = (uint32_t)(g - (size_t)y * W);
        const uint32_t blk = y / rb;
        uint32_t rank, lb;
        share_owner(blk, nranks, share, rank, lb);
        const uint32_t ly = lb * rb + (y - blk * rb);
        out[g] = gathered[((size_t)rank * shard_rows + ly) * W + x];
    }
}

#ifdef VR_EXPERIMENTS
static uint32_t march_lds_pad()
{
    static const uint32_t v = [] {
        const char *e = std::getenv("VR_MARCH_LDS_PAD");
        return e ? (uint32_t)std::strtoul(e, nullptr, 10) : 0u;
    }();
    return v;
}
#else
constexpr uint32_t march_lds_pad() { return 0; }
#endif

using VariantTypes = std::tuple<uint8_t, int8_t, uint16_t, int16_t, float, Quad8<uint8_t>,
                                Quad8<int8_t>, F32Alt, F32H, F32P, F32S>;
static_assert(std::tuple_size<VariantTypes>::value == kVariantTags, "one type per VariantTag");
using FrameLauncher = void (*)(uint32_t nblocks, const MarchParams &, const MipArgs &, const IsoArgs &,
                               hipStream_t);

template <int I>
void launch_slot(uint32_t nblocks, const MarchParams &p, const MipArgs &m, const IsoArgs &iso,
                 hipStream_t stream)
{
    constexpr FrameVariant v = variant_at(I);
    using VT = std::tuple_element_t<v.tag, VariantTypes>;
    if constexpr (v.family == VF_MARCH)
        hipLaunchKernelGGL((march_kernel<VT, v.shade, v.count, v.skip, v.gf, v.pipe>), dim3(nblocks),
                           dim3(kThreadsPerTile), march_lds_pad(), stream, p);
    else if constexpr (v.family == VF_PAIR)
        hipLaunchKernelGGL((march_pair_kernel<VT, v.shade, v.gf, v.lanes>), dim3(nblocks),
                           dim3(kThreads), 0, stream, p);
    else if constexpr (v.family == VF_MIP)
        hipLaunchKernelGGL((mip_kernel<VT, v.count, v.skip, v.inflight>), dim3(nblocks),
                           dim3(kThreadsPerTile), 0, stream, p, m);
    else
        hipLaunchKernelGGL((iso_kernel<VT, v.count, v.skip, v.inflight>), dim3(nblocks),
                           dim3(kThreadsPerTile), 0, stream, p, iso);
}

template <int I>
constexpr FrameLauncher slot_launcher()
{
    if constexpr (variant_built(variant_at(I)) && variant_index(variant_at(I)) == I)
        return &launch_slot<I>;
    else
        return nullptr;
}
template <int... I>
constexpr std::array<FrameLauncher, sizeof...(I)> slot_launchers(std::integer_sequence<int, I...>)
{
    return {{slot_launcher<I>()...}};
}

inline unsigned grid_bricks(size_t nb)
{
    return (unsigned)(nb > 65536 ? 65536 : (nb == 0 ? 1 : nb));
}

inline unsigned grid_for(size_t total)
{
    size_t g = (total + 255) / 256;
    return (unsigned)(g > 2048 * 8 ? 2048 * 8 : (g == 0 ? 1 : g));
}

template <typename T>
__global__ __launch_bounds__(256) void unbrick_kernel(const Vox<T> *__restrict__ bricks,
                                                     Vox<T> *__restrict__ dst, uint32_t nx,
                                                     uint32_t ny, uint32_t nbx, uint32_t nby,
                                                     uint32_t z0, size_t count)
{
    constexpr size_t vpe = std::is_same<T, float>::value ? kF32VoxelsPerElement
                                                         : (kPlainByte<T> ? 1 : 4);
    for (size_t g = (size_t)blockIdx.x * blockDim.x + threadIdx.x; g < count;
         g += (size_t)gridDim.x * blockDim.x) {
        const uint32_t x = (uint32_t)(g % nx);
        const size_t yz = g / nx;
        const uint32_t y = (uint32_t)(yz % ny), z = z0 + (uint32_t)(yz / ny);
        const uint32_t pi = x + kPad, pj = y + kPad, pk = z + kPad;
        dst[g] = bricks[cell_offset<T>((int)pi, (int)pj, (int)pk, nbx, nby) * vpe];
    }
}

template <typename SrcT>
hipError_t brick_from(const void *src, void *dst, uint32_t nx, uint32_t ny, uint32_t nz,
                      int storage, hipStream_t s)
{
    const uint32_t nbx = bricks_for(nx, 0, storage), nby = bricks_for(ny, 1, storage),
                   nbz = bricks_for(nz, 2, storage);
    const size_t total = (size_t)nbx * nby * nbz;
    const SrcT *sp = static_cast<const SrcT *>(src);
    switch (storage) {
        case ST_U8: hipLaunchKernelGGL((brick_kernel<SrcT, uint8_t>), dim3(grid_bricks(total)), dim3(256), 0, s, sp, (uint8_t *)dst, nx, ny, nz, nbx, nby, total); break;
        case ST_I8: hipLaunchKernelGGL((brick_kernel<SrcT, int8_t>), dim3(grid_bricks(total)), dim3(256), 0, s, sp, (int8_t *)dst, nx, ny, nz, nbx, nby, total); break;
        case ST_U8 | kQuadFlag: hipLaunchKernelGGL((brick_kernel<SrcT, Quad8<uint8_t>>), dim3(grid_bricks(total)), dim3(256), 0, s, sp, (uint8_t *)dst, nx, ny, nz, nbx, nby, total); break;
        case ST_I8 | kQuadFlag: hipLaunchKernelGGL((brick_kernel<SrcT, Quad8<int8_t>>), dim3(grid_bricks(total)), dim3(256), 0, s, sp, (int8_t *)dst, nx, ny, nz, nbx, nby, total); break;
        case ST_U16: hipLaunchKernelGGL((brick_kernel<SrcT, uint16_t>), dim3(grid_bricks(total)), dim3(256), 0, s, sp, (uint16_t *)dst, nx, ny, nz, nbx, nby, total); break;
        case ST_I16: hipLaunchKernelGGL((brick_kernel<SrcT, int16_t>), dim3(grid_bricks(total)), dim3(256), 0, s, sp, (int16_t *)dst, nx, ny, nz, nbx, nby, total); break;
        case ST_F32 | kAltFlag: hipLaunchKernelGGL((brick_kernel<SrcT, F32Alt>), dim3(grid_bricks(total)), dim3(256), 0, s, sp, (float *)dst, nx, ny, nz, nbx, nby, total); break;
        case ST_F32 | kPlainF32Flag: hipLaunchKernelGGL((brick_kernel<SrcT, F32P>), dim3(grid_bricks(total)), dim3(256), 0, s, sp, (float *)dst, nx, ny, nz, nbx, nby, total); break;
        case ST_F32 | kStencilF32Flag: hipLaunchKernelGGL((brick_kernel<SrcT, F32S>), dim3(grid_bricks(total)), dim3(256), 0, s, sp, (float *)dst, nx, ny, nz, nbx, nby, total); break;
        default: hipLaunchKernelGGL((brick_kernel<SrcT, float>), dim3(grid_bricks(total)), dim3(256), 0, s, sp, (float *)dst, nx, ny, nz, nbx, nby, total); break;
    }
    return hipGetLastError();
}

}

hipError_t launch_frame(const FrameVariant &v, const MarchParams &p, const MipArgs &m,
                        const IsoArgs &iso, hipStream_t stream)
{
    static constexpr auto launchers = slot_launchers(std::make_integer_sequence<int, kVariantSlots>{});
// ... 75 lines not shown
        case ST_U16: hipLaunchKernelGGL((minmax_kernel<uint16_t>), dim3(g), dim3(256), 0, s, (const uint16_t *)linear, count, o); break;
        case ST_I16: hipLaunchKernelGGL((minmax_kernel<int16_t>), dim3(g), dim3(256), 0, s, (const int16_t *)linear, count, o); break;
        default: hipLaunchKernelGGL((minmax_kernel<float>), dim3(g), dim3(256), 0, s, (const float *)linear, count, o); break;
    }
    return hipGetLastError();
}

hipError_t launch_int_range(int src_dtype, const void *src, size_t count, int *out3_dev,
                            hipStream_t s)
{
    const unsigned g = std::min(grid_for(count), 2048u);
    switch (src_dtype) {
        case 5: hipLaunchKernelGGL((int_range_kernel<int32_t>), dim3(g), dim3(256), 0, s, (const int32_t *)src, count, out3_dev); break;
        case 6: hipLaunchKernelGGL((int_range_kernel<uint32_t>), dim3(g), dim3(256), 0, s, (const uint32_t *)src, count, out3_dev); break;
        case 7: hipLaunchKernelGGL((int_range_kernel<int64_t>), dim3(g), dim3(256), 0, s, (const int64_t *)src, count, out3_dev); break;
        case 8: hipLaunchKernelGGL((int_range_kernel<uint64_t>), dim3(g), dim3(256), 0, s, (const uint64_t *)src, count, out3_dev); break;
        case 9: hipLaunchKernelGGL((int_range_kernel<float>), dim3(g), dim3(256), 0, s, (const float *)src, count, out3_dev); break;
        default: return hipErrorInvalidValue;
    }
    return hipGetLastError();
}

hipError_t launch_assemble(const void *gathered, void *out, int out_format, uint32_t W,
                           uint32_t H, uint32_t row_block, uint32_t nranks,
                           uint32_t shard_rows, RowShare share, hipStream_t s)
{
    const unsigned g = grid_for((size_t)W * H);
    if (out_format == 0)
        hipLaunchKernelGGL((assemble_kernel<uint32_t>), dim3(g), dim3(256), 0, s,
                           (const uint32_t *)gathered, (uint32_t *)out, W, H, row_block, nranks,
                           shard_rows, share);
    else
        hipLaunchKernelGGL((assemble_kernel<float4>), dim3(g), dim3(256), 0, s,
                           (const float4 *)gathered, (float4 *)out, W, H, row_block, nranks,
                           shard_rows, share);
    return hipGetLastError();
}

hipError_t launch_brick_range(int storage, const void *bricks, uint32_t nbx, uint32_t nby,
                              uint32_t nbz, float2 *range_dev, hipStream_t s)
{
    const uint32_t nbricks = nbx * nby * nbz;
    const unsigned g = (nbricks + 3) / 4;
    const uint32_t per = (uint32_t)(brick_elems(storage) * voxels_per_element(storage));
    switch (storage & 0xF) {
        case ST_U8: hipLaunchKernelGGL((brick_range_kernel<uint8_t>), dim3(g), dim3(256), 0, s, (const uint8_t *)bricks, nbricks, per, nbx, nby, range_dev); break;
        case ST_I8: hipLaunchKernelGGL((brick_range_kernel<int8_t>), dim3(g), dim3(256), 0, s, (const int8_t *)bricks, nbricks, per, nbx, nby, range_dev); break;
        case ST_U16: hipLaunchKernelGGL((brick_range_kernel<uint16_t>), dim3(g), dim3(256), 0, s, (const uint16_t *)bricks, nbricks, per, nbx, nby, range_dev); break;
        case ST_I16: hipLaunchKernelGGL((brick_range_kernel<int16_t>), dim3(g), dim3(256), 0, s, (const int16_t *)bricks, nbricks, per, nbx, nby, range_dev); break;
        default: hipLaunchKernelGGL((brick_range_kernel<float>), dim3(g), dim3(256), 0, s, (const float *)bricks, nbricks, per, nbx, nby, range_dev); break;
    }
    return hipGetLastError();
}

hipError_t launch_grad_field(const float *bricks, float *grad, uint32_t nx, uint32_t ny,
                             uint32_t nz, bool half, int scale_log2, hipStream_t s)
{
    const uint32_t nbx = bricks_for(nx, 0, ST_F32), nby = bricks_for(ny, 1, ST_F32),
                   nbz = bricks_for(nz, 2, ST_F32);
    const size_t total = (size_t)nbx * nby * nbz;
    const float scale = std::ldexp(1.0f, scale_log2);
    if (half)
        hipLaunchKernelGGL(grad_field_kernel<true>, dim3(grid_bricks(total)), dim3(256), 0, s,
                           bricks, grad, nx, ny, nz, nbx, nby, total, scale);
    else
        hipLaunchKernelGGL(grad_field_kernel<false>, dim3(grid_bricks(total)), dim3(256), 0, s,
                           bricks, grad, nx, ny, nz, nbx, nby, total, scale);
    return hipGetLastError();
}

hipError_t launch_rebrick_f32(const float *src_bricks, void *dst, uint32_t nx, uint32_t ny,
                              uint32_t nz, int storage, hipStream_t s)
{
    const uint32_t snbx = bricks_for(nx, 0, ST_F32), snby = bricks_for(ny, 1, ST_F32),
                   snbz = bricks_for(nz, 2, ST_F32);
    const uint32_t nbx = bricks_for(nx, 0, storage), nby = bricks_for(ny, 1, storage),
                   nbz = bricks_for(nz, 2, storage);
    const size_t total = (size_t)nbx * nby * nbz;
    float *d = static_cast<float *>(dst);
    switch (storage) {
        case ST_F32 | kAltFlag: hipLaunchKernelGGL((rebrick_f32_kernel<F32Alt>), dim3(grid_bricks(total)), dim3(256), 0, s, src_bricks, d, nx, ny, nz, snbx, snby, snbz, nbx, nby, total); break;
        case ST_F32 | kPlainF32Flag: hipLaunchKernelGGL((rebrick_f32_kernel<F32P>), dim3(grid_bricks(total)), dim3(256), 0, s, src_bricks, d, nx, ny, nz, snbx, snby, snbz, nbx, nby, total); break;
        case ST_F32 | kStencilF32Flag: hipLaunchKernelGGL((rebrick_f32_kernel<F32S>), dim3(grid_bricks(total)), dim3(256), 0, s, src_bricks, d, nx, ny, nz, snbx, snby, snbz, nbx, nby, total); break;
        default: return hipErrorInvalidValue;
    }
    return hipGetLastError();
}

hipError_t launch_skip_dist(const float2 *range_dev, uint32_t nbx, uint32_t nby, uint32_t nbz,
                            const uint32_t *tf_nz_dev, int tf_n, float vmin, float vrange,
                            uint8_t *dist_dev, uint8_t *scratch_dev, hipStream_t s)
{
    const uint32_t nb = nbx * nby * nbz;
    const unsigned g = (nb + 255) / 256;
    hipLaunchKernelGGL(classify_kernel, dim3(g), dim3(256), 0, s, range_dev, nb, tf_nz_dev, tf_n,
                       (float)tf_n, vmin, vrange, dist_dev);
    hipLaunchKernelGGL(dist_pass_kernel, dim3(g), dim3(256), 0, s, (const uint8_t *)dist_dev,
                       scratch_dev, nbx, nby, nbz, 0);
    hipLaunchKernelGGL(dist_pass_kernel, dim3(g), dim3(256), 0, s, (const uint8_t *)scratch_dev,
                       dist_dev, nbx, nby, nbz, 1);
    hipLaunchKernelGGL(dist_pass_kernel, dim3(g), dim3(256), 0, s, (const uint8_t *)dist_dev,
                       scratch_dev, nbx, nby, nbz, 2);
    return hipMemcpyAsync(dist_dev, scratch_dev, nb, hipMemcpyDeviceToDevice, s);
}

#ifdef VR_WG_TIMES
hipError_t debug_wg_times_reset()
{
    const unsigned int z = 0;
    return hipMemcpyToSymbol(HIP_SYMBOL(g_wg_count), &z, sizeof(z));
}
hipError_t debug_wg_times_read(unsigned long long *out, unsigned int max, unsigned int *count)
{
    unsigned int n = 0;
    hipError_t e = hipMemcpyFromSymbol(&n, HIP_SYMBOL(g_wg_count), sizeof(n));
    if (e != hipSuccess) return e;
    n = n < kWgTimesMax ? n : kWgTimesMax;
    n = n < max ? n : max;
    *count = n;
    return n ? hipMemcpyFromSymbol(out, HIP_SYMBOL(g_wg_times), 4 * n * sizeof(unsigned long long))
             : hipSuccess;
}
#endif

hipError_t launch_order_tiles(const uint32_t *cost, const uint32_t *lists, uint32_t *perm,
                              uint32_t per_xcd, hipStream_t s)
{
    hipLaunchKernelGGL(order_tiles_kernel, dim3(8), dim3(256), 0, s, cost, lists, perm, per_xcd);
    return hipGetLastError();
}

}
```

volumetric-renderer_amd/csrc/vr_variant.h:

```cpp
#pragma once

#include <stdint.h>

#include <string>

#include "../../include/vr/vr_debug.h"
#include "../../include/vr/vr_modes.h"

namespace vr {

enum StorageType { ST_U8 = 0, ST_I8 = 1, ST_U16 = 2, ST_I16 = 3, ST_F32 = 4 };
constexpr int kQuadFlag = 0x10, kAltFlag = 0x20, kPlainF32Flag = 0x100, kStencilF32Flag = 0x200;
constexpr int kTfLds = 256;

enum VariantFamily { VF_NONE = -1, VF_MARCH = 0, VF_PAIR = 1, VF_MIP = 2, VF_ISO = 3 };
enum VariantTag {
    TAG_U8, TAG_I8, TAG_U16, TAG_I16, TAG_F32, TAG_QUAD_U8, TAG_QUAD_I8,
    TAG_F32ALT, TAG_F32H, TAG_F32P, TAG_F32S, kVariantTags
};
constexpr const char *kTagNames[kVariantTags] = {
    "unsigned char", "signed char", "unsigned short", "short", "float",
    "vr::Quad8<unsigned char>", "vr::Quad8<signed char>", "vr::F32Alt", "vr::F32H", "vr::F32P",
    "vr::F32S"};

struct FrameVariant {
    int family = VF_NONE, tag = 0;
    bool shade = false, count = false, skip = false, gf = false, pipe = false;
    int lanes = 0;
    int inflight = 0;
};

using VariantFacts = ::vr_variant_facts;

inline bool resolve_variant(const VariantFacts &f, FrameVariant *v)
{
    *v = FrameVariant{};
    const int base = f.layout >= ST_U8 && f.layout <= ST_F32 ? f.layout
                     : f.layout == (ST_U8 | kQuadFlag)       ? TAG_QUAD_U8
                     : f.layout == (ST_I8 | kQuadFlag)       ? TAG_QUAD_I8
                                                             : -1;
    const int alt = f.layout == (ST_F32 | kAltFlag)          ? TAG_F32ALT
                    : f.layout == (ST_F32 | kPlainF32Flag)   ? TAG_F32P
                    : f.layout == (ST_F32 | kStencilF32Flag) ? TAG_F32S
                                                             : -1;
    if (f.mode == VR_MODE_MIP || f.mode == VR_MODE_ISO) {
        const int k = f.count ? 1 : f.mip_inflight;
        if (base < 0 || (k != 1 && k != 2 && k != 4)) return false;
        *v = {f.mode == VR_MODE_ISO ? VF_ISO : VF_MIP, base, false, f.count != 0, f.skip != 0, false,
              false, 0, k};
        return true;
    }
    if (base < 0 && (alt < 0 || f.count || f.pair || f.skip || f.field)) return false;
    const bool gf = base == TAG_F32 && f.shade && f.field;
    const int tag = alt >= 0 ? alt : gf && f.field_half ? (int)TAG_F32H : base;
    if (f.pair)
        *v = {VF_PAIR, tag, f.shade != 0, false, false, gf, false, f.pair == 4 ? 4 : 2, 0};
    else
        *v = {VF_MARCH, tag, f.shade != 0, f.count != 0, f.skip != 0, gf,
              f.pipeline && !f.count && !f.skip && f.tf_n <= kTfLds, 0, 0};
    return true;
}

constexpr bool variant_built(const FrameVariant &v)
{
    const bool alt = v.tag == TAG_F32ALT || v.tag == TAG_F32P || v.tag == TAG_F32S;
    const bool field_type = v.tag == TAG_F32 || v.tag == TAG_F32H;
    if (v.tag < 0 || v.tag >= kVariantTags) return false;
    if (v.gf ? !(v.shade && field_type) : v.tag == TAG_F32H) return false;
    switch (v.family) {
        case VF_MARCH: return !(v.pipe && (v.count || v.skip)) && !(alt && (v.count || v.skip));
        case VF_PAIR: return !alt && (v.lanes == 2 || v.lanes == 4);
        case VF_MIP:
        case VF_ISO: return !alt && (v.inflight == 1 || (!v.count && (v.inflight == 2 || v.inflight == 4)));
        default: return false;
    }
}

constexpr int kVariantSlots = 4 * kVariantTags * 32;
constexpr int variant_index(const FrameVariant &v)
{
    const int k = v.inflight == 1 ? 0 : v.inflight == 2 ? 1 : v.inflight == 4 ? 2 : 3;
    const int bits = v.family == VF_MARCH  ? v.shade << 4 | v.count << 3 | v.skip << 2 | v.gf << 1 | (int)v.pipe
                     : v.family == VF_PAIR ? v.shade << 2 | v.gf << 1 | (v.lanes == 4)
                                           : v.count << 3 | v.skip << 2 | k;
    return (v.family * kVariantTags + v.tag) * 32 + bits;
}
constexpr FrameVariant variant_at(int i)
{
    const int family = i / 32 / kVariantTags, tag = i / 32 % kVariantTags;
    const auto bit = [i](int b) { return (i >> b & 1) != 0; };
    if (family == VF_MARCH) return {family, tag, bit(4), bit(3), bit(2), bit(1), bit(0), 0, 0};
    if (family == VF_PAIR) return {family, tag, bit(2), false, false, bit(1), false, bit(0) ? 4 : 2, 0};
    return {family, tag, false, bit(3), bit(2), false, false, 0, (i & 3) == 3 ? 0 : 1 << (i & 3)};
}

inline std::string variant_kernel_name(const FrameVariant &v)
{
    const auto b = [](bool x) { return x ? ", true" : ", false"; };
    if (v.family == VF_NONE || v.tag < 0 || v.tag >= kVariantTags) return "";
    const std::string ns = "void vr::(anonymous namespace)::", vt = kTagNames[v.tag];
    if (v.family == VF_MARCH)
        return ns + "march_kernel<" + vt + b(v.shade) + b(v.count) + b(v.skip) + b(v.gf) +
               b(v.pipe) + ">(vr::MarchParams)";
    if (v.family == VF_PAIR)
        return ns + "march_pair_kernel<" + vt + b(v.shade) + b(v.gf) + ", " +
               std::to_string(v.lanes) + ">(vr::MarchParams)";
    return ns + (v.family == VF_ISO ? "iso_kernel<" : "mip_kernel<") + vt + b(v.count) + b(v.skip) +
           ", " + std::to_string(v.inflight) +
           (v.family == VF_ISO ? ">(vr::MarchParams, vr::IsoArgs)" : ">(vr::MarchParams, vr::MipArgs)");
}

constexpr uint32_t variant_tile_key(const FrameVariant &v, int layout)
{
    static_assert(kVariantSlots <= 1 << 12, "the variant index and the layout would overlap");
    return (uint32_t)variant_index(v) | (uint32_t)layout << 12;
}

}
```

volumetric-renderer_amd/vr_amd.py:

```python
from __future__ import annotations

import contextlib
import ctypes as C
import os
from dataclasses import dataclass
from typing import Optional, Sequence

import numpy as np

HERE = os.path.dirname(os.path.abspath(__file__))
LIB_PATH = os.environ.get("VR_AMD_LIB") or os.path.join(HERE, "lib", "libvr_amd.so")

DTYPE_I8, DTYPE_U8, DTYPE_I16, DTYPE_U16, DTYPE_I32, DTYPE_U32 = 1, 2, 3, 4, 5, 6
DTYPE_I64, DTYPE_U64, DTYPE_F32, DTYPE_F64 = 7, 8, 9, 10
NP_TO_DTYPE = {
    np.dtype(np.int8): DTYPE_I8, np.dtype(np.uint8): DTYPE_U8,
    np.dtype(np.int16): DTYPE_I16, np.dtype(np.uint16): DTYPE_U16,
    np.dtype(np.int32): DTYPE_I32, np.dtype(np.uint32): DTYPE_U32,
    np.dtype(np.int64): DTYPE_I64, np.dtype(np.uint64): DTYPE_U64,
    np.dtype(np.float32): DTYPE_F32, np.dtype(np.float64): DTYPE_F64,
}
DTYPE_TO_NP = {v: k for k, v in NP_TO_DTYPE.items()}
STORAGE_BYTES = {0: 1, 1: 1, 2: 2, 3: 2, 4: 4}

OUT_RGBA8, OUT_RGBA32F = 0, 1


class vr_camera(C.Structure):
    _fields_ = [("view", C.c_float * 16), ("position", C.c_float * 3),
                ("fovy_deg", C.c_float), ("znear", C.c_float), ("zfar", C.c_float)]


class vr_params(C.Structure):
    _fields_ = [("step", C.c_float), ("ray_dist", C.c_float), ("ert_eps", C.c_float),
                ("shading", C.c_int32), ("clear_color", C.c_float * 4),
                ("ambient", C.c_float), ("diffuse", C.c_float), ("specular", C.c_float),
                ("spec_power", C.c_int32), ("tile_order", C.c_int32),
                ("skip_empty", C.c_int32), ("wave_shape", C.c_int32),
                ("frames_in_flight", C.c_int32), ("exact_gradient", C.c_int32),
                ("depth_zero_to_one", C.c_int32)]


class vr_stats(C.Structure):
    _fields_ = [("rays", C.c_uint64), ("samples", C.c_uint64),
                ("shaded_samples", C.c_uint64), ("steps", C.c_uint64),
                ("skipped_samples", C.c_uint64)]


class vr_orbit_camera(C.Structure):
    _fields_ = [("center", C.c_float * 3), ("orientation", C.c_float * 4),
                ("radius", C.c_float)]


class vr_memory_info(C.Structure):
    _fields_ = [(n, C.c_uint64) for n in (
        "volume_bytes", "field_bytes", "oblique_copy_bytes", "plain_copy_bytes",
        "stencil_copy_bytes", "skip_bytes", "derived_bytes", "budget_bytes",
        "builds", "evictions", "downgrades", "last_downgrade")]


class vr_dist_host_profile(C.Structure):
    _fields_ = [("frames", C.c_uint64)] + [(n, C.c_double) for n in (
        "render_us", "gather_us", "assemble_us", "record_us", "wait_us", "total_us")]


DERIVED = {1: "field", 2: "oblique_copy", 3: "plain_copy", 4: "stencil_copy", 5: "skip"}


class vr_member_timing(C.Structure):
    _fields_ = [("device", C.c_int32), ("frames", C.c_uint64), ("kernel_ms", C.c_double),
                ("render_ms", C.c_double), ("gather_ms", C.c_double), ("assemble_ms", C.c_double)]


class vr_variant_facts(C.Structure):
    _fields_ = [(n, C.c_int32) for n in (
        "layout", "mode", "shade", "count", "skip", "field", "field_half", "pipeline", "tf_n",
        "pair", "mip_inflight")]


class vr_dataset(C.Structure):
    _fields_ = [("dims", C.c_uint32 * 3), ("dtype", C.c_int), ("data", C.c_void_p),
                ("vmin", C.c_float), ("vmax", C.c_float)]


ABI_SYMBOLS = [
    "vr_abi_version", "vr_params_default", "vr_create", "vr_destroy", "vr_last_error",
    "vr_create_mask", "vr_get_device_mask",
    "vr_resize", "vr_get_size", "vr_get_device", "vr_set_volume", "vr_set_volume_device", "vr_generate_volume",
    "vr_volume_bytes", "vr_debug_read_volume", "vr_debug_read_volume_native", "vr_debug_volume_info",
    "vr_set_transfer_function", "vr_set_slicing", "vr_render", "vr_render_device",
    "vr_shard_rows", "vr_assemble_rows", "vr_count_work", "vr_timing_enable",
    "vr_timing_read", "vr_timing_reset", "vr_kernel_name",
    "vr_import_memory_fd", "vr_release_external_memory",
    "vr_set_row_share", "vr_get_row_share", "vr_shard_rows_ctx",
    "vr_set_memory_budget", "vr_memory_report", "vr_prepare",
]
HOST_SYMBOLS = [
    "vr_cam_init", "vr_cam_rotate", "vr_cam_zoom", "vr_cam_position", "vr_cam_view",
    "vr_cam_to_camera", "vr_gradient_create", "vr_gradient_destroy",
    "vr_gradient_add_color_marker", "vr_gradient_add_alpha_marker",
    "vr_gradient_remove_color_marker", "vr_gradient_remove_alpha_marker",
    "vr_gradient_set_alpha_marker", "vr_gradient_set_color_marker", "vr_gradient_marker_count",
    "vr_gradient_sample", "vr_gradient_discretize", "vr_nrrd_load", "vr_nrrd_write_raw",
    "vr_csv_load", "vr_dataset_free", "vr_host_last_error",
]

DIST_SYMBOLS = [
    "vr_dist_unique_id", "vr_dist_create", "vr_dist_render", "vr_dist_synchronize",
    "vr_dist_last_error", "vr_dist_destroy", "vr_dist_timing_enable", "vr_dist_timing_read",
    "vr_dist_host_profile_enable", "vr_dist_host_profile_read",
]
DIST_ID_BYTES = 128
DEBUG_SYMBOLS = ["vr_debug_set_knob", "vr_debug_get_knob", "vr_debug_timing_member",
                 "vr_debug_create_members", "vr_debug_fail_member",
                 "vr_debug_host_profile_enable", "vr_debug_host_profile_member",
                 "vr_debug_variant_name", "vr_debug_last_kernel_name"]
MODES_SYMBOLS = ["vr_set_render_mode", "vr_get_render_mode"]
MODE_COMPOSITE, MODE_MIP = 0, 1
MODE_ISO = 3
ISO_SYMBOLS = ["vr_set_isovalue", "vr_get_isovalue"]
EXCHANGE_RCCL, EXCHANGE_COPY = 0, 1
KNOBS = {"pipeline": 1, "pair": 2, "pair_lanes": 3, "grad_field": 4, "u8_layout": 6,
         "tile_order": 7, "narrow": 8, "alt_geometry": 9, "mip_inflight": 10}
KNOB_AUTO = {"pipeline": -1, "pair": -1, "pair_lanes": 0, "grad_field": -1,
             "u8_layout": -1, "tile_order": 0, "narrow": 1, "alt_geometry": -1,
             "mip_inflight": 0}

ABI_VERSION = 9
_LIB = None


def lib() -> C.CDLL:
    global _LIB
    if _LIB is not None:
        return _LIB
    if not os.path.exists(LIB_PATH):
        raise RuntimeError(f"{LIB_PATH} is missing: build it with `make -C volumetric-renderer_amd` "
                           "(or __graft_entry__.build()); there is no CPU fallback")
    try:
        import torch
    except ImportError:
        pass
    L = C.CDLL(LIB_PATH)
    vp, u32, f32, i32 = C.c_void_p, C.c_uint32, C.c_float, C.c_int
    sig = {
        "vr_abi_version": (i32, []),
        "vr_params_default": (None, [C.POINTER(vr_params)]),
        "vr_create": (vp, [i32, u32, u32]),
        "vr_destroy": (None, [vp]),
        "vr_last_error": (C.c_char_p, [vp]),
        "vr_resize": (i32, [vp, u32, u32]),
        "vr_get_size": (i32, [vp, C.POINTER(u32), C.POINTER(u32)]),
        "vr_get_device": (i32, [vp, C.POINTER(i32)]),
        "vr_create_mask": (vp, [u32, u32, u32]),
        "vr_get_device_mask": (i32, [vp, C.POINTER(u32)]),
        "vr_dist_unique_id": (i32, [vp]),
        "vr_dist_create": (vp, [vp, vp, i32, i32, u32, i32]),
        "vr_dist_render": (i32, [vp, C.POINTER(vr_camera), C.POINTER(vr_params), vp, vp]),
        "vr_dist_synchronize": (i32, [vp]),
        "vr_dist_last_error": (C.c_char_p, [vp]),
        "vr_dist_destroy": (None, [vp]),
        "vr_dist_timing_enable": (i32, [vp, i32]),
        "vr_dist_host_profile_enable": (i32, [vp, i32]),
        "vr_dist_host_profile_read": (i32, [vp, C.POINTER(vr_dist_host_profile)]),
        "vr_dist_timing_read": (i32, [vp, C.POINTER(C.c_double), C.POINTER(C.c_double),
                                      C.POINTER(C.c_uint64)]),
        "vr_set_volume": (i32, [vp, vp, i32, u32, u32, u32, f32, f32]),
        "vr_set_volume_device": (i32, [vp, vp, i32, u32, u32, u32, f32, f32, vp]),
        "vr_generate_volume": (i32, [vp, i32, i32, u32, u32, u32, u32, C.POINTER(f32), C.POINTER(f32)]),
        "vr_volume_bytes": (C.c_uint64, [vp]),
        "vr_debug_read_volume": (i32, [vp, vp]),
        "vr_debug_read_volume_native": (i32, [vp, vp]),
        "vr_debug_volume_info": (i32, [vp, C.POINTER(u32), C.POINTER(f32), C.POINTER(i32)]),
        "vr_set_transfer_function": (i32, [vp, C.POINTER(u32), u32]),
        "vr_set_slicing": (i32, [vp, C.POINTER(f32), C.POINTER(f32)]),
        "vr_render": (i32, [vp, C.POINTER(vr_camera), C.POINTER(vr_params), vp, i32]),
        "vr_render_device": (i32, [vp, C.POINTER(vr_camera), C.POINTER(vr_params), vp, i32, u32, u32, u32, vp]),
        "vr_shard_rows": (u32, [u32, u32, u32]),
        "vr_assemble_rows": (i32, [vp, vp, vp, i32, u32, u32, vp]),
        "vr_count_work": (i32, [vp, C.POINTER(vr_camera), C.POINTER(vr_params), u32, u32, u32, C.POINTER(vr_stats)]),
        "vr_timing_enable": (i32, [vp, i32]),
        "vr_timing_read": (i32, [vp, C.POINTER(C.c_double), C.POINTER(C.c_uint64)]),
        "vr_timing_reset": (i32, [vp]),
        "vr_kernel_name": (C.c_char_p, [vp, C.POINTER(vr_params)]),
        "vr_import_memory_fd": (C.c_int, [vp, C.c_int, C.c_uint64, C.c_uint64, C.POINTER(vp),
                                          C.POINTER(vp)]),
        "vr_release_external_memory": (C.c_int, [vp, vp]),
        "vr_debug_set_knob": (i32, [vp, i32, i32]),
        "vr_debug_timing_member": (i32, [vp, i32, C.POINTER(vr_member_timing)]),
        "vr_debug_host_profile_enable": (i32, [vp, i32]),
        "vr_debug_host_profile_member": (i32, [vp, i32, C.POINTER(vr_dist_host_profile)]),
        "vr_set_row_share": (i32, [vp, u32, u32]),
        "vr_get_row_share": (i32, [vp, C.POINTER(u32), C.POINTER(u32)]),
        "vr_shard_rows_ctx": (u32, [vp, u32, u32, u32]),
        "vr_set_memory_budget": (i32, [vp, C.c_uint64]),
        "vr_memory_report": (i32, [vp, C.POINTER(vr_memory_info)]),
        "vr_prepare": (i32, [vp, C.POINTER(vr_camera), C.POINTER(vr_params)]),
        "vr_debug_get_knob": (i32, [vp, i32, C.POINTER(i32)]),
        "vr_set_render_mode": (i32, [vp, i32]),
        "vr_get_render_mode": (i32, [vp, C.POINTER(i32)]),
        "vr_set_isovalue": (i32, [vp, C.c_float]),
        "vr_get_isovalue": (i32, [vp, C.POINTER(C.c_float)]),
        "vr_debug_create_members": (vp, [C.POINTER(i32), i32, u32, u32, i32]),
        "vr_debug_fail_member": (i32, [vp, i32, C.c_uint64]),
        "vr_debug_variant_name": (i32, [C.POINTER(vr_variant_facts), C.c_char_p, C.c_size_t]),
        "vr_debug_last_kernel_name": (C.c_char_p, [vp]),
        "vr_cam_init": (None, [C.POINTER(vr_orbit_camera)]),
        "vr_cam_rotate": (None, [C.POINTER(vr_orbit_camera), f32, f32]),
        "vr_cam_zoom": (None, [C.POINTER(vr_orbit_camera), f32]),
        "vr_cam_position": (None, [C.POINTER(vr_orbit_camera), C.POINTER(f32)]),
        "vr_cam_view": (None, [C.POINTER(vr_orbit_camera), C.POINTER(f32)]),
        "vr_cam_to_camera": (None, [C.POINTER(vr_orbit_camera), C.POINTER(vr_camera)]),
        "vr_gradient_create": (vp, []),
        "vr_gradient_destroy": (None, [vp]),
        "vr_gradient_add_color_marker": (i32, [vp, f32, f32, f32, f32]),
        "vr_gradient_add_alpha_marker": (i32, [vp, f32, f32]),
        "vr_gradient_remove_color_marker": (i32, [vp, C.c_size_t]),
        "vr_gradient_remove_alpha_marker": (i32, [vp, C.c_size_t]),
        "vr_gradient_set_alpha_marker": (i32, [vp, C.c_size_t, f32, f32]),
        "vr_gradient_set_color_marker": (i32, [vp, C.c_size_t, f32, f32, f32, f32]),
        "vr_gradient_marker_count": (C.c_size_t, [vp, i32]),
        "vr_gradient_sample": (None, [vp, f32, C.POINTER(f32)]),
        "vr_gradient_discretize": (i32, [vp, C.c_size_t, C.POINTER(u32)]),
        "vr_nrrd_load": (i32, [C.c_char_p, C.POINTER(vr_dataset)]),
        "vr_nrrd_write_raw": (i32, [C.c_char_p, vp, i32, C.POINTER(u32)]),
        "vr_csv_load": (i32, [C.POINTER(C.c_char_p), C.c_size_t, C.POINTER(vr_dataset)]),
        "vr_dataset_free": (None, [C.POINTER(vr_dataset)]),
        "vr_host_last_error": (C.c_char_p, []),
    }
    for name, (res, args) in sig.items():
        fn = getattr(L, name)
        fn.restype = res
        fn.argtypes = args
    if L.vr_abi_version() != ABI_VERSION:
        raise RuntimeError(f"{LIB_PATH} has ABI {L.vr_abi_version()}, this binding expects "
                           f"{ABI_VERSION}: rebuild it")
    _LIB = L
    return L


def default_params(**overrides) -> vr_params:
    p = vr_params()
    lib().vr_params_default(C.byref(p))
    for k, v in overrides.items():
        if k == "clear_color":
            for i in range(4):
                p.clear_color[i] = v[i]
        else:
            setattr(p, k, v)
    return p


class OrbitCamera:

    def __init__(self):
        self._c = vr_orbit_camera()
        lib().vr_cam_init(C.byref(self._c))

    def rotate(self, dx: float, dy: float) -> "OrbitCamera":
        lib().vr_cam_rotate(C.byref(self._c), dx, dy)
        return self

    def zoom(self, delta: float) -> "OrbitCamera":
        lib().vr_cam_zoom(C.byref(self._c), delta)
        return self

    def set_radius(self, r: float) -> "OrbitCamera":
        self._c.radius = r
        return self

    @property
    def radius(self) -> float:
        return float(self._c.radius)

    def get_position(self) -> np.ndarray:
        out = (C.c_float * 3)()
        lib().vr_cam_position(C.byref(self._c), out)
        return np.array(out[:], dtype=np.float32)

    def get_view(self) -> np.ndarray:
        out = (C.c_float * 16)()
        lib().vr_cam_view(C.byref(self._c), out)
        return np.array(out[:], dtype=np.float32)

    def to_vr_camera(self) -> vr_camera:
        cam = vr_camera()
        lib().vr_cam_to_camera(C.byref(self._c), C.byref(cam))
        return cam

# ... 215 lines not shown
        v = C.c_float()
        self._check(lib().vr_get_isovalue(self._ctx, C.byref(v)), "vr_get_isovalue")
        return float(v.value)

    def render(self, camera: OrbitCamera, params: Optional[vr_params] = None,
               out_format: int = OUT_RGBA32F, out: Optional[np.ndarray] = None) -> np.ndarray:
        w, h = self.size
        p = params if params is not None else default_params()
        cam = camera.to_vr_camera() if isinstance(camera, OrbitCamera) else camera
        dt = np.float32 if out_format == OUT_RGBA32F else np.uint8
        if out is None:
            out = np.empty((h, w, 4), dtype=dt)
        elif out.shape != (h, w, 4) or out.dtype != dt or not out.flags.c_contiguous:
            raise ValueError(f"out must be a C-contiguous ({h}, {w}, 4) {np.dtype(dt).name} array")
        self._check(lib().vr_render(self._ctx, C.byref(cam), C.byref(p), out.ctypes.data, out_format),
                    "render")
        return out

    def render_device(self, camera, params, out_ptr: int, out_format: int = OUT_RGBA8,
                      row_block: int = 16, rank: int = 0, nranks: int = 1, stream: int = 0):
        cam = camera.to_vr_camera() if isinstance(camera, OrbitCamera) else camera
        self._check(lib().vr_render_device(self._ctx, C.byref(cam), C.byref(params),
                                           C.c_void_p(out_ptr), out_format, row_block, rank,
                                           nranks, C.c_void_p(stream or None)), "render_device")

    def assemble_rows(self, gathered_ptr: int, out_ptr: int, out_format: int, row_block: int,
                      nranks: int, stream: int = 0):
        self._check(lib().vr_assemble_rows(self._ctx, C.c_void_p(gathered_ptr), C.c_void_p(out_ptr),
                                           out_format, row_block, nranks, C.c_void_p(stream or None)),
                    "assemble_rows")

    def count_work(self, camera, params, row_block=16, rank=0, nranks=1) -> dict:
        cam = camera.to_vr_camera() if isinstance(camera, OrbitCamera) else camera
        st = vr_stats()
        self._check(lib().vr_count_work(self._ctx, C.byref(cam), C.byref(params), row_block, rank,
                                        nranks, C.byref(st)), "count_work")
        return dict(rays=st.rays, samples=st.samples, shaded_samples=st.shaded_samples,
                    steps=st.steps, skipped_samples=st.skipped_samples)

    def timing_enable(self, on: bool = True):
        self._check(lib().vr_timing_enable(self._ctx, 1 if on else 0), "timing_enable")

    def timing_read(self):
        ms, n = C.c_double(), C.c_uint64()
        self._check(lib().vr_timing_read(self._ctx, C.byref(ms), C.byref(n)), "timing_read")
        return float(ms.value), int(n.value)

    def timing_reset(self):
        self._check(lib().vr_timing_reset(self._ctx), "timing_reset")

    def kernel_name(self, params) -> str:
        return lib().vr_kernel_name(self._ctx, C.byref(params)).decode()

    def last_kernel_name(self) -> str:
        return lib().vr_debug_last_kernel_name(self._ctx).decode()

    def timing_member(self, member: int) -> dict:
        t = vr_member_timing()
        self._check(lib().vr_debug_timing_member(self._ctx, member, C.byref(t)), "timing_member")
        return dict(device=int(t.device), frames=int(t.frames), kernel_ms=float(t.kernel_ms),
                    render_ms=float(t.render_ms), gather_ms=float(t.gather_ms),
                    assemble_ms=float(t.assemble_ms))

    def fail_member(self, member: int, frame: int):
        self._check(lib().vr_debug_fail_member(self._ctx, member, frame), "vr_debug_fail_member")

    def set_row_share(self, first_weight: int, other_weight: int):
        self._check(lib().vr_set_row_share(self._ctx, first_weight, other_weight), "set_row_share")

    def row_share(self):
        a, b = C.c_uint32(), C.c_uint32()
        self._check(lib().vr_get_row_share(self._ctx, C.byref(a), C.byref(b)), "row_share")
        return int(a.value), int(b.value)

    def shard_rows(self, height: int, row_block: int, nranks: int) -> int:
        return int(lib().vr_shard_rows_ctx(self._ctx, height, row_block, nranks))

    def set_memory_budget(self, nbytes: int):
        self._check(lib().vr_set_memory_budget(self._ctx, C.c_uint64(nbytes)), "set_memory_budget")

    def memory_report(self) -> dict:
        m = vr_memory_info()
        self._check(lib().vr_memory_report(self._ctx, C.byref(m)), "memory_report")
        return {n: int(getattr(m, n)) for n, _ in vr_memory_info._fields_}

    def prepare(self, camera, params):
        cam = camera.to_vr_camera() if isinstance(camera, OrbitCamera) else camera
        self._check(lib().vr_prepare(self._ctx, C.byref(cam), C.byref(params)), "prepare")

    def host_profile_enable(self, on: bool = True):
        self._check(lib().vr_debug_host_profile_enable(self._ctx, int(bool(on))), "host_profile_enable")

    def host_profile_member(self, member: int) -> dict:
        h = vr_dist_host_profile()
        self._check(lib().vr_debug_host_profile_member(self._ctx, member, C.byref(h)),
                    "host_profile_member")
        n = max(int(h.frames), 1)
        return dict(frames=int(h.frames), **{k: getattr(h, k) / n for k, _ in vr_dist_host_profile._fields_[1:]})

    def set_knob(self, name: str, value: int):
        self._check(lib().vr_debug_set_knob(self._ctx, KNOBS[name], int(value)), f"set_knob({name})")

    def get_knob(self, name: str) -> int:
        v = C.c_int()
        self._check(lib().vr_debug_get_knob(self._ctx, KNOBS[name], C.byref(v)), f"get_knob({name})")
        return int(v.value)

    @contextlib.contextmanager
    def knobs(self, **kw):
        for k, v in kw.items():
            self.set_knob(k, v)
        try:
            yield self
        finally:
            for k in kw:
                self.set_knob(k, KNOB_AUTO[k])


def dist_unique_id() -> bytes:
    buf = C.create_string_buffer(DIST_ID_BYTES)
    rc = lib().vr_dist_unique_id(buf)
    if rc:
        raise RuntimeError(f"vr_dist_unique_id failed ({rc}): {lib().vr_dist_last_error(None).decode()}")
    return buf.raw


class DistFrames:

    def __init__(self, rp: "OffscreenPass", uid: bytes, nranks: int, rank: int,
                 row_block: int = 8, frames_in_flight: int = 3):
        if len(uid) != DIST_ID_BYTES:
            raise ValueError("communicator id must be DIST_ID_BYTES bytes")
        self.rank, self.nranks = rank, nranks
        self._rp = rp
        self._d = lib().vr_dist_create(rp._ctx, C.create_string_buffer(uid, DIST_ID_BYTES),
                                       nranks, rank, row_block, frames_in_flight)
        if not self._d:
            raise RuntimeError(f"vr_dist_create failed: {lib().vr_dist_last_error(None).decode()}")

    def _check(self, rc: int, what: str):
        if rc:
            raise RuntimeError(f"{what} failed ({rc}): {lib().vr_dist_last_error(self._d).decode()}")

    def render(self, camera, params, frame_ptr: int = 0, stream: int = 0):
        cam = camera.to_vr_camera() if isinstance(camera, OrbitCamera) else camera
        self._check(lib().vr_dist_render(self._d, C.byref(cam), C.byref(params),
                                         C.c_void_p(frame_ptr or None), C.c_void_p(stream or None)),
                    "vr_dist_render")

    def synchronize(self):
        self._check(lib().vr_dist_synchronize(self._d), "vr_dist_synchronize")

    def timing_enable(self, on: bool = True):
        self._check(lib().vr_dist_timing_enable(self._d, 1 if on else 0), "vr_dist_timing_enable")

    def host_profile(self, enable=None):
        if enable is not None:
            self._check(lib().vr_dist_host_profile_enable(self._d, 1 if enable else 0),
                        "vr_dist_host_profile_enable")
            return None
        h = vr_dist_host_profile()
        self._check(lib().vr_dist_host_profile_read(self._d, C.byref(h)), "vr_dist_host_profile_read")
        n = max(int(h.frames), 1)
        return dict(frames=int(h.frames), **{k: getattr(h, k) / n for k, _ in vr_dist_host_profile._fields_[1:]})

    def timing_read(self):
        r, g, n = C.c_double(), C.c_double(), C.c_uint64()
        self._check(lib().vr_dist_timing_read(self._d, C.byref(r), C.byref(g), C.byref(n)),
                    "vr_dist_timing_read")
        return r.value, g.value, n.value

    def close(self):
        if getattr(self, "_d", None):
            lib().vr_dist_destroy(self._d)
            self._d = None

    def __del__(self):
        try:
            self.close()
        except Exception:
            pass


KERNEL_SOURCES = ("csrc/vr_kernels.hip", "csrc/vr_internal.h", "csrc/vr_exact_math.h", "Makefile")


def kernel_source_hash() -> str:
    import hashlib
    h = hashlib.sha256()
    for rel in KERNEL_SOURCES:
        with open(os.path.join(HERE, rel), "rb") as f:
            h.update(f.read())
    return h.hexdigest()[:16]


def _elf_sections(b: bytes, base: int = 0):
    import struct
    shoff = struct.unpack_from("<Q", b, base + 0x28)[0]
    shentsize, shnum, shstrndx = struct.unpack_from("<HHH", b, base + 0x3A)
    secs = [struct.unpack_from("<IIQQQQIIQQ", b, base + shoff + i * shentsize) for i in range(shnum)]
    names = base + secs[shstrndx][4]
    return [(b[names + s[0]:b.index(b"\0", names + s[0])],) + s for s in secs]


def code_object_symbols(path: Optional[str] = None):
    import re
    import struct
    b = open(path or LIB_PATH, "rb").read()
    fb = [s for s in _elf_sections(b) if s[0] == b".hip_fatbin"]
    if not fb:
        raise RuntimeError(f"{path or LIB_PATH} has no .hip_fatbin section")
    fat = b[fb[0][5]:fb[0][5] + fb[0][6]]
    for p in (m.start() for m in re.finditer(b"__CLANG_OFFLOAD_BUNDLE__", fat)):
        q = p + 32
        for _ in range(struct.unpack_from("<Q", fat, p + 24)[0]):
            off, size, tl = struct.unpack_from("<QQQ", fat, q)
            triple = fat[q + 24:q + 24 + tl]
            q += 24 + tl
            if b"gfx950" not in triple:
                continue
            co = fat[p + off:p + off + size]
            secs = _elf_sections(co)
            st = next(s for s in secs if s[0] == b".symtab")
            strt = next(s for s in secs if s[0] == b".strtab")
            for i in range(st[6] // 24):
                nm, _, _, shndx, val, sz = struct.unpack_from("<IBBHQQ", co, st[5] + i * 24)
                name = co[strt[5] + nm:co.index(b"\0", strt[5] + nm)]
                if 0 < shndx < len(secs) and sz > 0:
                    sec = secs[shndx]
                    code = bytearray(co[sec[5] + val - sec[4]:sec[5] + val - sec[4] + sz])
                    if name.endswith(b".kd") and len(code) >= 24:
                        code[16:24] = bytes(8)
                    yield name, bytes(code)


def kernel_code_hash(path: Optional[str] = None) -> str:
    import hashlib
    syms = [(name, code) for name, code in code_object_symbols(path)
            if any(k in name for k in (b"12march_kernel", b"17march_pair_kernel",
                                       b"18order_tiles_kernel"))]
    if not syms:
        raise RuntimeError(f"{path or LIB_PATH}: no march_kernel code in the gfx950 code object")
    h = hashlib.sha256()
    for name, code in sorted(syms):
        h.update(name)
        h.update(code)
    return h.hexdigest()[:16]


def variant_name(**facts) -> Optional[str]:
    buf = C.create_string_buffer(256)
    f = vr_variant_facts(**facts)
    return buf.value.decode() if lib().vr_debug_variant_name(C.byref(f), buf, len(buf)) == 0 else None


def shard_rows(height: int, row_block: int, nranks: int) -> int:
    return int(lib().vr_shard_rows(height, row_block, nranks))


def unorm8(img: np.ndarray) -> np.ndarray:
    v = np.clip(np.nan_to_num(img.astype(np.float32), nan=0.0), np.float32(0), np.float32(1))
    return np.floor(v * np.float32(255.0) + np.float32(0.5)).astype(np.uint8)
```

Measured before the change: 367.0.

## Add y-major brick copy and march_y kernel for y-axis rays on large volumes

Adds a derived volume copy whose bricks are stored y-major, so rays marching mainly along y read contiguous memory. A dedicated march_y_kernel with a matching decode and a rebrick kernel are added, and the variant tables, memory accounting and knob range are extended. The copy is chosen only when knobs are at default, rows are dense, the ray axis is y and the volume exceeds the assumed 256 MiB Infinity Cache. The extra copy costs memory and a one-time rebrick, and it is the first derived copy evicted when room is needed.

```diff
diff --git a/include/vr/vr.h b/include/vr/vr.h
--- a/include/vr/vr.h
+++ b/include/vr/vr.h
@@ -137,7 +137,8 @@
     VR_DERIVED_OBLIQUE_COPY = 2,
     VR_DERIVED_PLAIN_COPY = 3,
     VR_DERIVED_STENCIL_COPY = 4,
-    VR_DERIVED_SKIP = 5
+    VR_DERIVED_SKIP = 5,
+    VR_DERIVED_YMAJOR_COPY = 6
 };
 #define VR_MEMORY_BUDGET_UNLIMITED (~(uint64_t)0)
 #define VR_MEMORY_BUDGET_DEFAULT (~(uint64_t)0 - 1)
diff --git a/include/vr/vr_debug.h b/include/vr/vr_debug.h
--- a/include/vr/vr_debug.h
+++ b/include/vr/vr_debug.h
@@ -46,6 +46,8 @@
 int vr_debug_variant_name(const vr_variant_facts *facts, char *buf, size_t n);
 const char *vr_debug_last_kernel_name(const vr_ctx *ctx);
 
+uint64_t vr_debug_ymajor_copy_bytes(const vr_ctx *ctx);
+
 #ifdef __cplusplus
 }
 #endif
diff --git a/volumetric-renderer_amd/csrc/vr_api.hip b/volumetric-renderer_amd/csrc/vr_api.hip
--- a/volumetric-renderer_amd/csrc/vr_api.hip
+++ b/volumetric-renderer_amd/csrc/vr_api.hip
@@ -40,7 +40,7 @@
         size_t bytes = 0;
         bool valid = false, failed = false;
         uint64_t used = 0;
-    } alt[3];
+    } alt[4];
     uint32_t nx = 1, ny = 1, nz = 1;
     float vmin = 0.0f, vmax = 1.0f;
     float4 *tf = nullptr;
@@ -519,7 +519,8 @@
            (shading && c->storage == ST_F32);
 }
 
-int want_alt(const vr_ctx *c, const vr_params *p, bool pair, bool field);
+int want_alt(const vr_ctx *c, const vr_params *p, bool pair, bool field, bool field_half,
+             bool pipelined);
 bool use_pair(const vr_ctx *c, const MarchParams &P, const vr_params *p)
 {
     if (p->skip_empty || P.tf_n > kTfLds) return false;
@@ -530,7 +531,8 @@
     if (c->knobs.alt >= 0 || c->layout != ST_F32 || c->dense_rows || c->pixel_span <= kAltSpan ||
         (c->ray_axis == 2 && c->axis_align >= kAltAlign))
         return false;
-    return want_alt(c, p, P.pair != 0, P.grad != nullptr) == (ST_F32 | kAltFlag);
+    return want_alt(c, p, P.pair != 0, P.grad != nullptr, P.grad_half != 0, P.pipelined != 0) ==
+           (ST_F32 | kAltFlag);
 }
 
 int build_params(vr_ctx *c, const vr_camera *cam, const vr_params *p, void *out,
@@ -703,6 +705,7 @@
     HIP_TRY(c, hipFreeAsync(p, s), "hipFreeAsync(derived structure)");
     return VR_OK;
 }
+constexpr int kYMajorAlt = 3;
 int make_room(vr_ctx *c, size_t extra, size_t replaced, int keep_alt, bool keep_field, hipStream_t s,
               bool *fits)
 {
@@ -719,6 +722,7 @@
                 pick = i;
                 oldest = c->alt[i].used;
             }
+        if (keep_alt != kYMajorAlt && c->alt[kYMajorAlt].bricks) pick = kYMajorAlt;
         if (pick == -2) return VR_OK;
         if (pick == -1) {
             if (int rc = release_async(c, c->grad, s)) return rc;
@@ -940,9 +944,27 @@
     return {M.brick_range, M.nbricks, c->isovalue, p->shading != 0};
 }
 
-int want_alt(const vr_ctx *c, const vr_params *p, bool pair, bool field)
-{
-    if (c->layout != ST_F32 || p->skip_empty || pair || field) return c->layout;
+constexpr size_t kInfinityCacheBytes = 256ull << 20;
+bool knobs_default(const vr_ctx *c)
+{
+    const vr_ctx::Knobs &k = c->knobs;
+    return k.pipeline < 0 && k.pair < 0 && k.pair_lanes == 0 && k.grad_field < 0 && k.alt < 0 &&
+           k.tile_order == 0;
+}
+bool want_ymajor(const vr_ctx *c, const vr_params *p, bool field, bool field_half, bool pipelined)
+{
+    if (!pipelined || c->tf_n > (uint32_t)kTfLds) return false;
+    if (p->shading ? !(field && field_half && p->exact_gradient == 0) : field) return false;
+    if (c->knobs.alt >= 0) return c->knobs.alt == 5;
+    return knobs_default(c) && c->dense_rows && c->ray_axis == 1 &&
+           c->brick_bytes > kInfinityCacheBytes;
+}
+int want_alt(const vr_ctx *c, const vr_params *p, bool pair, bool field, bool field_half,
+             bool pipelined)
+{
+    if (c->layout != ST_F32 || p->skip_empty || pair) return c->layout;
+    if (want_ymajor(c, p, field, field_half, pipelined)) return ST_F32 | kYMajorFlag;
+    if (field) return c->layout;
     int which = 0;
     if (c->knobs.alt >= 0)
         which = c->knobs.alt;
@@ -965,7 +987,13 @@
 int alt_index(int layout)
 {
     if (layout & kAltFlag) return 0;
+    if (layout & kYMajorFlag) return kYMajorAlt;
     return (layout & kPlainF32Flag) ? 1 : 2;
+}
+uint32_t alt_derived_code(int layout)
+{
+    return (layout & kYMajorFlag) ? (uint32_t)VR_DERIVED_YMAJOR_COPY
+                                  : (uint32_t)(VR_DERIVED_OBLIQUE_COPY + alt_index(layout));
 }
 
 size_t alt_bytes_for(const vr_ctx *c, int lay)
@@ -988,7 +1016,9 @@
     if (!a.bricks || a.bytes != bytes) {
         const size_t had = a.bricks ? a.bytes + kBrickSlackBytes : 0;
         bool fits = false;
-        if (int rc = make_room(c, bytes + kBrickSlackBytes, had, alt_index(lay), false, s, &fits))
+        if (lay & kYMajorFlag)
+            fits = budget_allows(c, bytes + kBrickSlackBytes, had);
+        else if (int rc = make_room(c, bytes + kBrickSlackBytes, had, alt_index(lay), false, s, &fits))
             return rc;
         if (!fits) return VR_OK;
         if (int rc = release_async(c, a.bricks, s)) return rc;
@@ -1042,8 +1072,8 @@
     f.field_half = f.field && p->exact_gradient == 0;
     const uint32_t tiles = ((c->width + 15) / 16) * ((c->height + kMarchRows - 1) / kMarchRows);
     f.pipeline = use_pipeline(f.shade, tiles, c);
-    if (p && !f.field)
-        if (const int lay = want_alt(c, p, false, false);
+    if (p)
+        if (const int lay = want_alt(c, p, false, f.field != 0, f.field_half != 0, f.pipeline != 0);
             lay != c->layout && c->alt[alt_index(lay)].valid)
             f.layout = lay;
     return f;
@@ -1198,7 +1228,7 @@
     switch (knob) {
         case VR_KNOB_PAIR_LANES: return v == 0 || v == 2 || v == 4;
         case VR_KNOB_NARROW: return v == 0 || v == 1;
-        case VR_KNOB_ALT_GEOMETRY: return v >= -1 && v <= 4 && v != 2;
+        case VR_KNOB_ALT_GEOMETRY: return v >= -1 && v <= 5 && v != 2;
         case VR_KNOB_TILE_ORDER: return v >= 0 && v <= 4;
         case VR_KNOB_MIP_INFLIGHT: return v == 0 || v == 1 || v == 2 || v == 4;
         default: return v >= -1 && v <= 1;
@@ -1961,7 +1991,9 @@
             P.tiles_y = (P.local_rows + th - 1) / th;
             P.supers_total = P.supers_x * ((P.tiles_y + kSuper - 1) / kSuper);
         }
-        if (const int lay = want_alt(c, p, P.pair != 0, P.grad != nullptr); lay != c->layout) {
+        if (const int lay = want_alt(c, p, P.pair != 0, P.grad != nullptr, P.grad_half != 0,
+                                     P.pipelined != 0);
+            lay != c->layout) {
             bool ready = false;
             rc = ensure_alt(c, lay, s, &ready);
             if (rc) return rc;
@@ -1972,7 +2004,7 @@
                 P.nbx = bricks_for(c->nx, 0, layout);
                 P.nby = bricks_for(c->ny, 1, layout);
             } else {
-                refused = (uint32_t)(VR_DERIVED_OBLIQUE_COPY + alt_index(lay));
+                if (!(lay & kYMajorFlag) || c->knobs.alt == 5) refused = alt_derived_code(lay);
             }
         }
     }
@@ -2354,6 +2386,14 @@
     return name.c_str();
 }
 
+uint64_t vr_debug_ymajor_copy_bytes(const vr_ctx *c)
+{
+    if (!c) return 0;
+    if (is_group(c)) return vr_debug_ymajor_copy_bytes(c->members[0]);
+    const vr_ctx::AltCopy &a = c->alt[kYMajorAlt];
+    return a.bricks ? a.bytes + kBrickSlackBytes : 0;
+}
+
 int vr_debug_set_knob(vr_ctx *c, int knob, int value)
 {
     if (!c) return fail(nullptr, VR_EINVAL, "ctx is NULL");
diff --git a/volumetric-renderer_amd/csrc/vr_internal.h b/volumetric-renderer_amd/csrc/vr_internal.h
--- a/volumetric-renderer_amd/csrc/vr_internal.h
+++ b/volumetric-renderer_amd/csrc/vr_internal.h
@@ -47,7 +47,7 @@
 constexpr int kGroupShift = VR_BRICK_GROUP_SHIFT;
 constexpr uint32_t kGroupMask = (1u << kGroupShift) - 1;
 
-__host__ __device__ __forceinline__ uint32_t morton_spread(uint32_t v)
+__host__ __device__ __forceinline__ constexpr uint32_t morton_spread(uint32_t v)
 {
     uint32_t r = 0;
 #pragma unroll
@@ -55,8 +55,9 @@
     return r;
 }
 
-__host__ __device__ __forceinline__ uint32_t brick_slot(uint32_t bx, uint32_t by, uint32_t bz,
-                                                        uint32_t nbx, uint32_t nby)
+__host__ __device__ __forceinline__ constexpr uint32_t brick_slot(uint32_t bx, uint32_t by,
+                                                                  uint32_t bz, uint32_t nbx,
+                                                                  uint32_t nby)
 {
     if constexpr (kGroupShift == 0) {
         return (bz * nby + by) * nbx + bx;
@@ -121,6 +122,68 @@
 struct F32H {
     float v;
 };
+struct F32Y {
+    float v;
+};
+struct F32HY {
+    float v;
+};
+__host__ __device__ constexpr uint32_t zmajor_local(uint32_t xl, uint32_t yl, uint32_t zl)
+{
+    return xl + (uint32_t)GeomWide::EX * (yl + (uint32_t)GeomWide::EY * zl);
+}
+__host__ __device__ constexpr uint32_t ymajor_local(uint32_t xl, uint32_t yl, uint32_t zl)
+{
+    return xl + (uint32_t)GeomWide::EX * (zl + (uint32_t)GeomWide::EZ * yl);
+}
+__host__ __device__ constexpr int ymajor_field_delta(uint32_t yl, uint32_t zl)
+{
+    return GeomWide::EX * (GeomWide::BY * (int)zl - GeomWide::BZ * (int)yl);
+}
+__host__ __device__ constexpr size_t ymajor_cell_offset(uint32_t pi, uint32_t pj, uint32_t pk,
+                                                        uint32_t nbx, uint32_t nby,
+                                                        int *field_delta = nullptr)
+{
+    using G = GeomWide;
+    const uint32_t bx = pi / G::BX, by = pj / G::BY, bz = pk / G::BZ;
+    const uint32_t xl = pi - bx * G::BX, yl = pj - by * G::BY, zl = pk - bz * G::BZ;
+    if (field_delta) *field_delta = ymajor_field_delta(yl, zl);
+    return (size_t)brick_slot(bx, by, bz, nbx, nby) * (size_t)G::Elems + ymajor_local(xl, yl, zl);
+}
+namespace ymajor_check {
+constexpr bool map_ok()
+{
+    using G = GeomWide;
+    constexpr uint32_t nbx = (3 + kGroupMask) & ~kGroupMask, nby = (2 + kGroupMask) & ~kGroupMask,
+                       nbz = nby;
+    for (uint32_t bz = 0; bz < nbz; ++bz)
+        for (uint32_t by = 0; by < nby; ++by)
+            for (uint32_t bx = 0; bx < nbx; ++bx) {
+                bool seen[G::EX * G::EY * G::EZ] = {};
+                const size_t base = (size_t)brick_slot(bx, by, bz, nbx, nby) * (size_t)G::Elems;
+                for (uint32_t zl = 0; zl < (uint32_t)G::EZ; ++zl)
+                    for (uint32_t yl = 0; yl < (uint32_t)G::EY; ++yl)
+                        for (uint32_t xl = 0; xl < (uint32_t)G::EX; ++xl) {
+                            const uint32_t l = ymajor_local(xl, yl, zl);
+                            if (l >= (uint32_t)(G::EX * G::EY * G::EZ) || seen[l]) return false;
+                            seen[l] = true;
+                            if ((int)zmajor_local(xl, yl, zl) - (int)l != ymajor_field_delta(yl, zl))
+                                return false;
+                            if (xl < (uint32_t)G::BX && yl < (uint32_t)G::BY && zl < (uint32_t)G::BZ) {
+                                int fd = 0;
+                                const size_t e = ymajor_cell_offset(bx * G::BX + xl, by * G::BY + yl,
+                                                                    bz * G::BZ + zl, nbx, nby, &fd);
+                                if (e != base + l || fd != ymajor_field_delta(yl, zl)) return false;
+                            }
+                        }
+            }
+    return true;
+}
+static_assert(map_ok(), "the y-major map is a bijection onto each brick, 72 (zl - yl) from z-major");
+static_assert(GeomWide::BX != 8 || GeomWide::BY != 8 || GeomWide::BZ != 8 ||
+                  ymajor_field_delta(3, 5) == 72 * (5 - 3),
+              "8^3 cells: l_zmajor - l_ymajor == 72 (zl - yl)");
+}
 
 inline size_t storage_size(int st)
 {
diff --git a/volumetric-renderer_amd/csrc/vr_kernels.hip b/volumetric-renderer_amd/csrc/vr_kernels.hip
--- a/volumetric-renderer_amd/csrc/vr_kernels.hip
+++ b/volumetric-renderer_amd/csrc/vr_kernels.hip
@@ -71,12 +71,22 @@
 struct VoxOf<F32S> {
     using type = float;
 };
+template <>
+struct VoxOf<F32Y> {
+    using type = float;
+};
+template <>
+struct VoxOf<F32HY> {
+    using type = float;
+};
 template <typename VT>
 using Vox = typename VoxOf<VT>::type;
 template <typename VT>
 constexpr bool kIsQuad8 = is_quad8<VT>::value;
 template <typename VT>
-constexpr bool kHalfField = std::is_same<VT, F32H>::value;
+constexpr bool kHalfField = std::is_same<VT, F32H>::value || std::is_same<VT, F32HY>::value;
+template <typename VT>
+constexpr bool kYMajor = std::is_same<VT, F32Y>::value || std::is_same<VT, F32HY>::value;
 template <typename VT>
 constexpr bool kZPair = std::is_same<Vox<VT>, float>::value;
 template <typename VT>
@@ -107,6 +117,7 @@
 {
     using G = GeomOf<VT>;
     const uint32_t ux = (uint32_t)pi, uy = (uint32_t)pj, uz = (uint32_t)pk;
+    if constexpr (kYMajor<VT>) return ymajor_cell_offset(ux, uy, uz, nbx, nby);
     const uint32_t bx = ux / G::BX, by = uy / G::BY, bz = uz / G::BZ;
     const uint32_t l = ((uz - bz * G::BZ + G::Lo) * G::EY + (uy - by * G::BY + G::Lo)) * G::EX +
                        (ux - bx * G::BX + G::Lo);
@@ -250,7 +261,16 @@
     }
     __device__ __forceinline__ void decode(const CellRaw<VT> &w)
     {
-        if constexpr (kZPair<VT> && !kPlainF32<VT>) {
+        if constexpr (kYMajor<VT>) {
+            v[0] = w.r0.x;
+            v[2] = w.r0.y;
+            v[1] = w.r0.z;
+            v[3] = w.r0.w;
+            v[4] = w.r1.x;
+            v[6] = w.r1.y;
+            v[5] = w.r1.z;
+            v[7] = w.r1.w;
+        } else if constexpr (kZPair<VT> && !kPlainF32<VT>) {
             v[0] = w.r0.x;
             v[4] = w.r0.y;
             v[1] = w.r0.z;
@@ -284,7 +304,7 @@
     }
     __device__ __forceinline__ void load(const char *__restrict__ base, size_t e)
     {
-        if constexpr (kStencilWide<VT>) {
+        if constexpr (kStencilWide<VT> || kYMajor<VT>) {
             CellRaw<VT> w;
             issue(w, base, e);
             decode(w);
@@ -975,9 +995,18 @@
             S.pi = i + kPad;
             S.pj = j + kPad;
             S.pk = kk + kPad;
-            S.ce = cell_offset<VT>(S.pi, S.pj, S.pk, P.nbx, P.nby);
-            if (VR_OOB(3, S.ce * kElemBytes<VT>, P.vol_bytes)) S.ce = 0;
-            Cell8<VT>::issue(S.w, vol, S.ce);
+            if constexpr (kYMajor<VT>) {
+                S.ce = cell_offset<float>(S.pi, S.pj, S.pk, P.nbx, P.nby);
+                size_t e = (size_t)((long)S.ce -
+                                    ymajor_field_delta((uint32_t)S.pj % (uint32_t)G::BY,
+                                                       (uint32_t)S.pk % (uint32_t)G::BZ));
+                if (VR_OOB(3, e * kElemBytes<VT>, P.vol_bytes)) e = S.ce = 0;
+                Cell8<VT>::issue(S.w, vol, e);
+            } else {
+                S.ce = cell_offset<VT>(S.pi, S.pj, S.pk, P.nbx, P.nby);
+                if (VR_OOB(3, S.ce * kElemBytes<VT>, P.vol_bytes)) S.ce = 0;
+                Cell8<VT>::issue(S.w, vol, S.ce);
+            }
         };
         auto composite = [&](const float4 &sm) -> bool {
             cr = cr + (sm.x * sm.w) * T;
@@ -1186,6 +1215,32 @@
     __syncthreads();
     if (tid == 0) wg_times_record((unsigned long long)wg_start, tile_y * P.tiles_x + tile_x);
 #endif
+}
+
+
+template <typename VT, bool SHADE>
+__global__ __launch_bounds__(kThreadsPerTile, (SHADE ? 6 : kMarchMinWaves<false, false, false, true>)) void march_y_kernel(const MarchParams P)
+{
+    static_assert(kYMajor<VT> && kHalfField<VT> == SHADE, "F32Y unshaded, F32HY shaded");
+    __shared__ float4 s_tf[kTfLut];
+    const int tid = threadIdx.x;
+
+    uint32_t tile_x, tile_y;
+    if (!block_tile(P, tile_x, tile_y)) return;
+    const long long wg_start = wall_clock64();
+
+    const bool tf_in_lds = P.tf_n <= kTfLds;
+    if (tf_in_lds)
+        for (int i = tid; i < 2 * (P.tf_n + 2); i += (int)kThreadsPerTile) s_tf[i] = P.tf[i];
+    __syncthreads();
+    march_strip<VT, SHADE, false, false, SHADE, true>(P, (LdsF4 *)s_tf, tf_in_lds, tile_x, tile_y,
+                                                      (uint32_t)tid >> 6, (uint32_t)tid & 63u);
+    if (P.tile_cost) {
+        __syncthreads();
+        if (tid == 0)
+            P.tile_cost[tile_y * P.tiles_x + tile_x] =
+                (uint32_t)min(wall_clock64() - wg_start, 0x7FFFFFFFLL);
+    }
 }
 
 template <typename VT>
@@ -1994,6 +2049,29 @@
     }
 }
 
+__global__ __launch_bounds__(256) void rebrick_ymajor_kernel(const float *__restrict__ src,
+                                                             float2 *__restrict__ dst, uint32_t nx,
+                                                             uint32_t ny, uint32_t nz, uint32_t nbx,
+                                                             uint32_t nby, size_t nbricks)
+{
+    using G = GeomWide;
+    for (size_t bidx = blockIdx.x; bidx < nbricks; bidx += gridDim.x) {
+        uint32_t bx, by, bz;
+        brick_coords((uint32_t)bidx, nbx, nby, bx, by, bz);
+        for (uint32_t l = threadIdx.x; l < (uint32_t)G::Elems; l += blockDim.x) {
+            const uint32_t lx = l % G::EX, lzy = l / G::EX, lz = lzy % G::EZ, ly = lzy / G::EZ;
+            float2 v = make_float2(0.0f, 0.0f);
+            if (ly < (uint32_t)G::EY) {
+                const int x = (int)(bx * G::BX + lx), y = (int)(by * G::BY + ly),
+                          z = (int)(bz * G::BZ + lz);
+                v = make_float2(padded_voxel(src, x, y, z, nx, ny, nz, nbx, nby),
+                                padded_voxel(src, x, y + 1, z, nx, ny, nz, nbx, nby));
+            }
+            dst[bidx * G::Elems + l] = v;
+        }
+    }
+}
+
 __device__ __forceinline__ _Float16 field_half(float d, float scale)
 {
     float x = d * scale;
@@ -2217,7 +2295,7 @@
 #endif
 
 using VariantTypes = std::tuple<uint8_t, int8_t, uint16_t, int16_t, float, Quad8<uint8_t>,
-                                Quad8<int8_t>, F32Alt, F32H, F32P, F32S>;
+                                Quad8<int8_t>, F32Alt, F32H, F32P, F32S, F32Y, F32HY>;
 static_assert(std::tuple_size<VariantTypes>::value == kVariantTags, "one type per VariantTag");
 using FrameLauncher = void (*)(uint32_t nblocks, const MarchParams &, const MipArgs &, const IsoArgs &,
                                hipStream_t);
@@ -2231,6 +2309,9 @@
     if constexpr (v.family == VF_MARCH)
         hipLaunchKernelGGL((march_kernel<VT, v.shade, v.count, v.skip, v.gf, v.pipe>), dim3(nblocks),
                            dim3(kThreadsPerTile), march_lds_pad(), stream, p);
+    else if constexpr (v.family == VF_MARCH_Y)
+        hipLaunchKernelGGL((march_y_kernel<VT, v.shade>), dim3(nblocks), dim3(kThreadsPerTile),
+                           march_lds_pad(), stream, p);
     else if constexpr (v.family == VF_PAIR)
         hipLaunchKernelGGL((march_pair_kernel<VT, v.shade, v.gf, v.lanes>), dim3(nblocks),
                            dim3(kThreads), 0, stream, p);
@@ -2472,6 +2553,7 @@
         case ST_F32 | kAltFlag: hipLaunchKernelGGL((rebrick_f32_kernel<F32Alt>), dim3(grid_bricks(total)), dim3(256), 0, s, src_bricks, d, nx, ny, nz, snbx, snby, snbz, nbx, nby, total); break;
         case ST_F32 | kPlainF32Flag: hipLaunchKernelGGL((rebrick_f32_kernel<F32P>), dim3(grid_bricks(total)), dim3(256), 0, s, src_bricks, d, nx, ny, nz, snbx, snby, snbz, nbx, nby, total); break;
         case ST_F32 | kStencilF32Flag: hipLaunchKernelGGL((rebrick_f32_kernel<F32S>), dim3(grid_bricks(total)), dim3(256), 0, s, src_bricks, d, nx, ny, nz, snbx, snby, snbz, nbx, nby, total); break;
+        case ST_F32 | kYMajorFlag: hipLaunchKernelGGL(rebrick_ymajor_kernel, dim3(grid_bricks(total)), dim3(256), 0, s, src_bricks, reinterpret_cast<float2 *>(d), nx, ny, nz, snbx, snby, total); break;
         default: return hipErrorInvalidValue;
     }
     return hipGetLastError();
diff --git a/volumetric-renderer_amd/csrc/vr_variant.h b/volumetric-renderer_amd/csrc/vr_variant.h
--- a/volumetric-renderer_amd/csrc/vr_variant.h
+++ b/volumetric-renderer_amd/csrc/vr_variant.h
@@ -10,18 +10,20 @@
 namespace vr {
 
 enum StorageType { ST_U8 = 0, ST_I8 = 1, ST_U16 = 2, ST_I16 = 3, ST_F32 = 4 };
-constexpr int kQuadFlag = 0x10, kAltFlag = 0x20, kPlainF32Flag = 0x100, kStencilF32Flag = 0x200;
+constexpr int kQuadFlag = 0x10, kAltFlag = 0x20, kPlainF32Flag = 0x100, kStencilF32Flag = 0x200,
+              kYMajorFlag = 0x400;
 constexpr int kTfLds = 256;
 
-enum VariantFamily { VF_NONE = -1, VF_MARCH = 0, VF_PAIR = 1, VF_MIP = 2, VF_ISO = 3 };
+enum VariantFamily { VF_NONE = -1, VF_MARCH = 0, VF_PAIR = 1, VF_MIP = 2, VF_ISO = 3, VF_MARCH_Y = 4 };
+constexpr int kVariantFamilies = 5;
 enum VariantTag {
     TAG_U8, TAG_I8, TAG_U16, TAG_I16, TAG_F32, TAG_QUAD_U8, TAG_QUAD_I8,
-    TAG_F32ALT, TAG_F32H, TAG_F32P, TAG_F32S, kVariantTags
+    TAG_F32ALT, TAG_F32H, TAG_F32P, TAG_F32S, TAG_F32Y, TAG_F32HY, kVariantTags
 };
 constexpr const char *kTagNames[kVariantTags] = {
     "unsigned char", "signed char", "unsigned short", "short", "float",
     "vr::Quad8<unsigned char>", "vr::Quad8<signed char>", "vr::F32Alt", "vr::F32H", "vr::F32P",
-    "vr::F32S"};
+    "vr::F32S", "vr::F32Y", "vr::F32HY"};
 
 struct FrameVariant {
     int family = VF_NONE, tag = 0;
@@ -43,6 +45,14 @@
                     : f.layout == (ST_F32 | kPlainF32Flag)   ? TAG_F32P
                     : f.layout == (ST_F32 | kStencilF32Flag) ? TAG_F32S
                                                              : -1;
+    if (f.layout == (ST_F32 | kYMajorFlag)) {
+        if (f.mode != VR_MODE_COMPOSITE || f.count || f.pair || f.skip || !f.pipeline ||
+            f.tf_n > kTfLds || (f.shade ? !(f.field && f.field_half) : f.field != 0))
+            return false;
+        *v = {VF_MARCH_Y, f.shade ? (int)TAG_F32HY : (int)TAG_F32Y, f.shade != 0, false, false,
+              f.shade != 0, true, 0, 0};
+        return true;
+    }
     if (f.mode == VR_MODE_MIP || f.mode == VR_MODE_ISO) {
         const int k = f.count ? 1 : f.mip_inflight;
         if (base < 0 || (k != 1 && k != 2 && k != 4)) return false;
@@ -66,6 +76,10 @@
     const bool alt = v.tag == TAG_F32ALT || v.tag == TAG_F32P || v.tag == TAG_F32S;
     const bool field_type = v.tag == TAG_F32 || v.tag == TAG_F32H;
     if (v.tag < 0 || v.tag >= kVariantTags) return false;
+    if (v.family == VF_MARCH_Y)
+        return v.tag == (v.shade ? TAG_F32HY : TAG_F32Y) && v.gf == v.shade && v.pipe && !v.count &&
+               !v.skip;
+    if (v.tag == TAG_F32Y || v.tag == TAG_F32HY) return false;
     if (v.gf ? !(v.shade && field_type) : v.tag == TAG_F32H) return false;
     switch (v.family) {
         case VF_MARCH: return !(v.pipe && (v.count || v.skip)) && !(alt && (v.count || v.skip));
@@ -76,11 +90,12 @@
     }
 }
 
-constexpr int kVariantSlots = 4 * kVariantTags * 32;
+constexpr int kVariantSlots = kVariantFamilies * kVariantTags * 32;
 constexpr int variant_index(const FrameVariant &v)
 {
     const int k = v.inflight == 1 ? 0 : v.inflight == 2 ? 1 : v.inflight == 4 ? 2 : 3;
-    const int bits = v.family == VF_MARCH  ? v.shade << 4 | v.count << 3 | v.skip << 2 | v.gf << 1 | (int)v.pipe
+    const bool march = v.family == VF_MARCH || v.family == VF_MARCH_Y;
+    const int bits = march                 ? v.shade << 4 | v.count << 3 | v.skip << 2 | v.gf << 1 | (int)v.pipe
                      : v.family == VF_PAIR ? v.shade << 2 | v.gf << 1 | (v.lanes == 4)
                                            : v.count << 3 | v.skip << 2 | k;
     return (v.family * kVariantTags + v.tag) * 32 + bits;
@@ -89,7 +104,8 @@
 {
     const int family = i / 32 / kVariantTags, tag = i / 32 % kVariantTags;
     const auto bit = [i](int b) { return (i >> b & 1) != 0; };
-    if (family == VF_MARCH) return {family, tag, bit(4), bit(3), bit(2), bit(1), bit(0), 0, 0};
+    if (family == VF_MARCH || family == VF_MARCH_Y)
+        return {family, tag, bit(4), bit(3), bit(2), bit(1), bit(0), 0, 0};
     if (family == VF_PAIR) return {family, tag, bit(2), false, false, bit(1), false, bit(0) ? 4 : 2, 0};
     return {family, tag, false, bit(3), bit(2), false, false, 0, (i & 3) == 3 ? 0 : 1 << (i & 3)};
 }
@@ -102,6 +118,8 @@
     if (v.family == VF_MARCH)
         return ns + "march_kernel<" + vt + b(v.shade) + b(v.count) + b(v.skip) + b(v.gf) +
                b(v.pipe) + ">(vr::MarchParams)";
+    if (v.family == VF_MARCH_Y)
+        return ns + "march_y_kernel<" + vt + b(v.shade) + ">(vr::MarchParams)";
     if (v.family == VF_PAIR)
         return ns + "march_pair_kernel<" + vt + b(v.shade) + b(v.gf) + ", " +
                std::to_string(v.lanes) + ">(vr::MarchParams)";
diff --git a/volumetric-renderer_amd/vr_amd.py b/volumetric-renderer_amd/vr_amd.py
--- a/volumetric-renderer_amd/vr_amd.py
+++ b/volumetric-renderer_amd/vr_amd.py
@@ -64,7 +64,8 @@
         "render_us", "gather_us", "assemble_us", "record_us", "wait_us", "total_us")]
 
 
-DERIVED = {1: "field", 2: "oblique_copy", 3: "plain_copy", 4: "stencil_copy", 5: "skip"}
+DERIVED = {1: "field", 2: "oblique_copy", 3: "plain_copy", 4: "stencil_copy", 5: "skip",
+           6: "ymajor_copy"}
 
 
 class vr_member_timing(C.Structure):
@@ -114,7 +115,8 @@
 DEBUG_SYMBOLS = ["vr_debug_set_knob", "vr_debug_get_knob", "vr_debug_timing_member",
                  "vr_debug_create_members", "vr_debug_fail_member",
                  "vr_debug_host_profile_enable", "vr_debug_host_profile_member",
-                 "vr_debug_variant_name", "vr_debug_last_kernel_name"]
+                 "vr_debug_variant_name", "vr_debug_last_kernel_name",
+                 "vr_debug_ymajor_copy_bytes"]
 MODES_SYMBOLS = ["vr_set_render_mode", "vr_get_render_mode"]
 MODE_COMPOSITE, MODE_MIP = 0, 1
 MODE_ISO = 3
@@ -205,6 +207,7 @@
         "vr_debug_fail_member": (i32, [vp, i32, C.c_uint64]),
         "vr_debug_variant_name": (i32, [C.POINTER(vr_variant_facts), C.c_char_p, C.c_size_t]),
         "vr_debug_last_kernel_name": (C.c_char_p, [vp]),
+        "vr_debug_ymajor_copy_bytes": (C.c_uint64, [vp]),
         "vr_cam_init": (None, [C.POINTER(vr_orbit_camera)]),
         "vr_cam_rotate": (None, [C.POINTER(vr_orbit_camera), f32, f32]),
         "vr_cam_zoom": (None, [C.POINTER(vr_orbit_camera), f32]),
@@ -586,7 +589,9 @@
     def memory_report(self) -> dict:
         m = vr_memory_info()
         self._check(lib().vr_memory_report(self._ctx, C.byref(m)), "memory_report")
-        return {n: int(getattr(m, n)) for n, _ in vr_memory_info._fields_}
+        r = {n: int(getattr(m, n)) for n, _ in vr_memory_info._fields_}
+        r["ymajor_copy_bytes"] = int(lib().vr_debug_ymajor_copy_bytes(self._ctx))
+        return r
 
     def prepare(self, camera, params):
         cam = camera.to_vr_camera() if isinstance(camera, OrbitCamera) else camera
@@ -741,8 +746,8 @@
 def kernel_code_hash(path: Optional[str] = None) -> str:
     import hashlib
     syms = [(name, code) for name, code in code_object_symbols(path)
-            if any(k in name for k in (b"12march_kernel", b"17march_pair_kernel",
-                                       b"18order_tiles_kernel"))]
+            if any(k in name for k in (b"12march_kernel", b"14march_y_kernel",
+                                       b"17march_pair_kernel", b"18order_tiles_kernel"))]
     if not syms:
         raise RuntimeError(f"{path or LIB_PATH}: no march_kernel code in the gfx950 code object")
     h = hashlib.sha256()
```

New measurement: 380.4 (median of 6 runs). 1.04x the previous value.
